# skit-ai/N-Best-ASR-Transformer

Measured on AMD Instinct MI355X. Metric: utterances/sec fine-tune (bert-base, seq128, n_best=5), higher is better.
Workload: dtype bf16

## Files before the change

include/nbest_hip.h:

```cpp
#ifndef NBEST_HIP_H
#define NBEST_HIP_H

#include <stddef.h>
#include <stdint.h>

#ifdef __cplusplus
extern "C" {
#endif

#define NBEST_ABI_VERSION 1

enum { NBEST_OK = 0, NBEST_ERR_ARG = -1, NBEST_ERR_SHAPE = -2, NBEST_ERR_DTYPE = -3, NBEST_ERR_ALIGN = -4,
       NBEST_ERR_LAUNCH = -5, NBEST_ERR_WORKSPACE = -6 };
enum { NBEST_F32 = 0, NBEST_BF16 = 1 };

typedef void* nbest_stream_t;

int nbest_version(void);
int nbest_last_error(char* buf, size_t n);

int nbest_embed_ln_fwd(const int64_t* ids, const int64_t* seg, const int64_t* pos, const void* word,
                       const void* type, const void* ptab, const float* gamma, const float* beta, void* out,
                       float* stats, int64_t M, int H, float eps, int dtype, float drop_p, uint64_t seed,
                       uint32_t drop_stream, nbest_stream_t stream);
int nbest_embed_ln_bwd(const int64_t* ids, const int64_t* seg, const int64_t* pos, const int32_t* perm, const void* word,
                       const void* type, const void* ptab, const float* gamma, const float* stats,
                       const void* dout, float* dword, float* dtype_tab, float* dptab, float* dgamma,
                       float* dbeta, int B, int S, int H, int n_types, int dtype, int64_t word_pad_id,
                       int64_t pos_pad_id, int accumulate, int tables_accumulate, float drop_p, uint64_t seed,
                       uint32_t drop_stream, void* ws, size_t ws_bytes, nbest_stream_t stream);
size_t nbest_embed_bwd_ws_bytes(int64_t M, int64_t H);
int nbest_embed_ln_fwd_interp(const int64_t* ids, const int64_t* base_ids, const float* alpha, const int64_t* seg, const int64_t* pos,
                              const void* word, const void* type, const void* ptab, const float* gamma, const float* beta, void* out,
                              float* stats, int B, int S, int H, float eps, int dtype, float drop_p, uint64_t seed, uint32_t drop_stream,
                              nbest_stream_t stream);
int nbest_embed_attrib(const int64_t* ids, const int64_t* base_ids, const float* alpha, const int64_t* seg, const int64_t* pos,
                       const void* word, const void* type, const void* ptab, const float* gamma, const void* dhidden, float* attr,
                       int pairs, int m, int S, int H, float eps, int dtype, nbest_stream_t stream);

int nbest_rows_gather(const float* table, const int64_t* rows, int64_t n_rows, int64_t cap, int64_t* ids_out, float* vals_out, int H,
                      nbest_stream_t stream);
int nbest_rows_zero(float* table, const int64_t* ids, int64_t n, int H, nbest_stream_t stream);
int nbest_rows_add(float* table, const int64_t* ids, const float* vals, int64_t n, int H, nbest_stream_t stream);

enum {
  NBEST_EPI_NONE = 0,
  NBEST_EPI_BIAS = 1,
  NBEST_EPI_BIAS_GELU = 2,
  NBEST_EPI_BIAS_DROP_RES = 3,
  NBEST_EPI_DGELU = 4,
  NBEST_EPI_RES = 5,
  NBEST_EPI_F32_SPLITK = 6
};
typedef struct nbest_gemm_args {
  const void* A;
  const void* B;
  void* C;
  const float* bias;
  const void* R;
  void* U;
  void* ws;
  size_t ws_bytes;
  int64_t M, N, K;
  int64_t lda, ldb, ldc, ldr, ldu;
  int32_t trans_a, trans_b;
  int32_t epilogue;
  int32_t dtype;
  int32_t accumulate;
  float drop_p;
  uint32_t drop_stream;
  uint64_t seed;
  float* colsum_out;
  int32_t colsum_accumulate;
  int32_t flags;
  const void* B_packed;
  int32_t b_pack_bn;
  int32_t pad_;
} nbest_gemm_args;
#define NBEST_GEMM_DEFER_REDUCE 1
size_t nbest_gemm_ws_bytes(const nbest_gemm_args* a);
int nbest_gemm(const nbest_gemm_args* a, nbest_stream_t stream);

size_t nbest_wgrad_pair_ws_bytes(const nbest_gemm_args* a, const nbest_gemm_args* b);
int nbest_wgrad_pair(const nbest_gemm_args* a, const nbest_gemm_args* b, nbest_stream_t stream);
int nbest_wgrad_group(const nbest_gemm_args* problems, int n, nbest_stream_t stream);

typedef struct nbest_gemm_fp8_args {
  const void* A;
  const void* B;
  void* C;
  const float* bias;
  const void* R;
  void* U;
  void* C8;
  int64_t M, N, K;
  int64_t lda, ldb, ldc, ldr, ldu, ldc8;
  int32_t epilogue;
  float out_scale;
  float drop_p;
  uint32_t drop_stream;
  uint64_t seed;
  const float* out_scale_dev;
  const uint32_t* a_amax;
  const uint32_t* c8_amax_prev;
  uint32_t* c8_amax_new;
  float* colsum_out;
  int32_t colsum_accumulate;
  int32_t pad;
  void* ws;
  size_t ws_bytes;
  const void* B_packed;
  int32_t b_pack_bn;
  int32_t pad3;
} nbest_gemm_fp8_args;
size_t nbest_gemm_fp8_ws_bytes(const nbest_gemm_fp8_args* a);
int nbest_gemm_fp8(const nbest_gemm_fp8_args* a, nbest_stream_t stream);
size_t nbest_wgrad_fp8_ws_bytes(int64_t M, int64_t N, int64_t K);
int nbest_wgrad_fp8(const void* dY8, const void* X8, float* dW, int64_t M, int64_t N, int64_t K, int64_t lda, int64_t ldb,
                    int64_t ldc, const uint32_t* a_amax, const uint32_t* x_amax, int accumulate, void* ws, size_t ws_bytes,
                    nbest_stream_t stream);
size_t nbest_wgrad_fp8_pair_ws_bytes(int64_t Ma, int64_t Mb, int64_t N, int64_t K);
int nbest_wgrad_fp8_pair(const void* dY8a, const void* X8a, float* dWa, int64_t Ma, int64_t lda_a, int64_t ldb_a, int64_t ldc_a,
                         const uint32_t* amax_a, const uint32_t* xamax_a, const void* dY8b, const void* X8b, float* dWb, int64_t Mb,
                         int64_t lda_b, int64_t ldb_b, int64_t ldc_b, const uint32_t* amax_b, const uint32_t* xamax_b, int64_t N, int64_t K,
                         int accumulate, void* ws, size_t ws_bytes, nbest_stream_t stream);
int nbest_cast_bf16_to_fp8(const void* src, void* dst, int64_t n, nbest_stream_t stream);

int nbest_attention_fwd(const void* qkv, const uint8_t* key_mask, void* ctx, float* lse, int B, int S,
                        int heads, int d, int dtype, float drop_p, uint64_t seed, uint32_t drop_stream,
                        nbest_stream_t stream);
int nbest_attention_cls_fwd(const void* q, int64_t ldq, const void* kv, int64_t ldkv, const uint8_t* key_mask, void* ctx,
                            int64_t ldctx, int B, int S, int heads, int d, int dtype, nbest_stream_t stream);
int nbest_attention_probs(const void* qkv, const uint8_t* key_mask, const float* lse, float* probs, int B, int S, int heads, int d,
                          int dtype, nbest_stream_t stream);
int nbest_attention_cls_probs(const void* q, int64_t ldq, const void* kv, int64_t ldkv, const uint8_t* key_mask, float* probs,
                              int64_t ldp, int B, int S, int heads, int d, int dtype, nbest_stream_t stream);
size_t nbest_attention_bwd_ws_bytes(int B, int S, int heads);
int nbest_attention_bwd(const void* qkv, const uint8_t* key_mask, const void* ctx, const void* dctx,
                        const float* lse, void* dqkv, float* dbias, int accumulate, void* ws, size_t ws_bytes,
                        int B, int S, int heads, int d, int dtype, float drop_p, uint64_t seed,
                        uint32_t drop_stream, nbest_stream_t stream);

size_t nbest_attention_keep_bytes(int B, int S, int heads);
int nbest_attention_fwd_keep(const void* qkv, const uint8_t* key_mask, void* ctx, float* lse, int B, int S,
                             int heads, int d, int dtype, float drop_p, uint64_t seed, uint32_t drop_stream,
                             void* keep, nbest_stream_t stream);
int nbest_attention_bwd_keep(const void* qkv, const uint8_t* key_mask, const void* ctx, const void* dctx,
                             const float* lse, void* dqkv, float* dbias, int accumulate, void* ws, size_t ws_bytes,
                             int B, int S, int heads, int d, int dtype, float drop_p, uint64_t seed,
                             uint32_t drop_stream, const void* keep, nbest_stream_t stream);

int nbest_layernorm_fwd(const void* x, const float* gamma, const float* beta, void* y, float* stats,
                        int64_t M, int H, float eps, int dtype, nbest_stream_t stream);
int nbest_layernorm_bwd(const void* dy, const void* x, const float* stats, const float* gamma, void* dx,
                        void* dx_drop, float* dgamma, float* dbeta, float* dbias, int64_t M, int H, int dtype,
                        int accumulate, float drop_p, uint64_t seed, uint32_t drop_stream, void* ws,
                        size_t ws_bytes, nbest_stream_t stream);
size_t nbest_rowred_ws_bytes(int64_t M, int64_t N);
int nbest_colsum(const void* X, float* out, int64_t M, int64_t N, int64_t ld, int dtype, int accumulate,
                 void* ws, size_t ws_bytes, nbest_stream_t stream);

typedef struct nbest_label_space {
  int32_t n_top, n_bottom, n_rows;
  const int32_t* bottom_off;
  const int32_t* bottom_ids;
  const int32_t* head_row;
} nbest_label_space;
size_t nbest_heads_ws_bytes(int B, int R, int H);
int nbest_stc_heads(const void* hidden, int64_t cls_stride, const float* Wh, const float* bh,
                    const nbest_label_space* ls, const float* labels, float* top, float* bott, float* final_scores,
                    float* loss_parts, float* dcls, float* dWh, float* dbh, int B, int H, int dtype,
                    int need_grad, int accumulate, float drop_p, uint64_t seed, uint32_t drop_stream, void* ws,
                    size_t ws_bytes, nbest_stream_t stream);
int nbest_stc_heads_vjp(const float* Wh, const nbest_label_space* ls, const float* top, const float* bott, const float* dtop,
                        const float* dbott, const float* dfin, float* dcls, float* dWh, float* dbh, int B, int H, int accumulate,
                        float drop_p, uint64_t seed, uint32_t drop_stream, void* ws, size_t ws_bytes, nbest_stream_t stream);

int nbest_cls_mse(const void* hidden_a, int64_t stride_a, const void* hidden_t, int64_t stride_t, float* loss,
                  float* da, float* dt, int B, int H, int dtype, float grad_scale, nbest_stream_t stream);

int nbest_cls_grad_scatter(const float* dcls, void* dhidden, int B, int S, int H, int dtype,
                           nbest_stream_t stream);

int nbest_stc_decode(const float* top, const float* bott, const nbest_label_space* ls,
                     const uint8_t* none_flag, int32_t* pred, int B, nbest_stream_t stream);
int nbest_stream_stamp(int32_t* flag, int32_t value, nbest_stream_t stream);

typedef struct nbest_tensor_desc {
  int64_t offset;
  int64_t numel;
  float lr;
  float wd;
  int32_t active;
  int32_t block_start;
} nbest_tensor_desc;
int nbest_bertadam_chunk(void);
int nbest_bertadam_step(float* p, float* g, float* m, float* v, void* p_lowp, const nbest_tensor_desc* descs,
                        int n_tensors, int n_blocks, float lr_mult, float b1, float b2, float eps,
                        float max_grad_norm, void* ws, size_t ws_bytes, nbest_stream_t stream);
int nbest_bertadam_norms(const float* g, const nbest_tensor_desc* descs, int n_tensors, int n_blocks, int blk_lo, int blk_hi,
                         float* partial, nbest_stream_t stream);
int nbest_bertadam_update(float* p, const float* g, float* m, float* v, void* p_lowp, const nbest_tensor_desc* descs,
                          int n_tensors, int n_blocks, int blk_lo, int blk_hi, const float* partial, float* coef,
                          float lr_mult, float b1, float b2, float eps, float max_grad_norm, nbest_stream_t stream);
enum { NBEST_ADAM_L2 = 0, NBEST_ADAMW = 1 };
int nbest_adam_clip_coef(const float* partial, int n_partial, float max_grad_norm, float* clip, nbest_stream_t stream);
int nbest_adam_update(int mode, float* p, const float* g, float* m, float* v, void* p_lowp, const nbest_tensor_desc* descs,
                      int n_tensors, int n_blocks, int blk_lo, int blk_hi, const float* clip, float lr_mult, float bc1,
                      float bc2_sqrt, double b1, double b2, float eps, nbest_stream_t stream);
int nbest_adam_step(int mode, float* p, float* g, float* m, float* v, void* p_lowp, const nbest_tensor_desc* descs,
                    int n_tensors, int n_blocks, float lr_mult, float bc1, float bc2_sqrt, double b1, double b2, float eps,
                    float max_grad_norm, void* ws, size_t ws_bytes, nbest_stream_t stream);
typedef struct nbest_matrix_desc {
  int64_t offset;
  int32_t rows, cols;
  int32_t tile_start, pad;
} nbest_matrix_desc;
#define NBEST_AMAX_TENSOR_WORDS 1024
int nbest_fp8_amax_fold(void* slots, void* out, int32_t n_tensors, nbest_stream_t stream);
int nbest_quantize_weights_fp8(const float* master, void* w8, void* w8t, const nbest_matrix_desc* descs, int n_matrices,
                               int n_tiles, float* inv_scale, void* ws, size_t ws_bytes, nbest_stream_t stream);
int nbest_transpose_weights(const void* src, void* dst, const nbest_matrix_desc* descs, int n_matrices, int n_tiles,
                            nbest_stream_t stream);
int nbest_pack_bn(int64_t N);
int nbest_pack_bn_fp8(int64_t N, int64_t K);
int nbest_pack_weights_fp8(const void* src, void* dst, const nbest_matrix_desc* descs, int n_matrices, int n_stages, nbest_stream_t stream);
int nbest_pack_weights(const void* src, void* dst, const nbest_matrix_desc* descs, int n_matrices, int n_stages, nbest_stream_t stream);
int nbest_cast_f32_to_bf16(const float* src, void* dst, int64_t n, nbest_stream_t stream);

typedef struct nbest_layer_offsets {
  int64_t wqkv, bqkv, wo, bo, ln1_g, ln1_b, w1, b1, w2, b2, ln2_g, ln2_b;
} nbest_layer_offsets;
typedef struct nbest_encoder_desc {
  int32_t dtype, B, S, H, L, heads, F;
  int32_t vocab, max_pos, n_types;
  float ln_eps, hidden_drop, attn_drop;
  int64_t word_pad_id, pos_pad_id;
  int64_t off_word, off_pos, off_type, off_emb_ln_g, off_emb_ln_b;
  const nbest_layer_offsets* layers_host;
  uint64_t seed;
  uint32_t drop_stream_base;
  int32_t wgrad_events_n;
  void** wgrad_events;
  const void* w8;
  const float* w8_inv_scale;
  const void* w8t;
  const uint32_t* gamax_prev;
  uint32_t* gamax_new;
  int32_t fp8_bwd;
  int32_t pad2;
  const void* wpk;
  const void* wpkt;
  const void* w8p;
  const void* w8tp;
  const int32_t* word_perm;
  const uint32_t* aamax_prev;
  uint32_t* aamax_new;
  int32_t fp8_act;
  int32_t pad4;
  int32_t first_trainable;
  int32_t no_input_grad;
  const uint8_t* wgrad_skip_host;
  const int64_t* base_ids;
  const float* alpha;
  int32_t no_param_grad;
  int32_t wgrad_group;
} nbest_encoder_desc;
enum { NBEST_WGRAD_GROUP_PLAN = 0, NBEST_WGRAD_GROUP_NEVER = 1, NBEST_WGRAD_GROUP_ALWAYS = 2 };
size_t nbest_encoder_act_bytes(const nbest_encoder_desc* d);
int nbest_encoder_act_view(const nbest_encoder_desc* d, void* act, int layer, void** qkv, float** lse);
size_t nbest_encoder_ws_bytes(const nbest_encoder_desc* d);
int nbest_encoder_wgrad_launches_per_layer(const nbest_encoder_desc* d);
int nbest_encoder_forward(const nbest_encoder_desc* d, const void* wts, const float* prm, const int64_t* ids,
                          const int64_t* seg, const int64_t* pos, const uint8_t* key_mask, void* act,
                          size_t act_bytes, void* ws, size_t ws_bytes, void** hidden_out, nbest_stream_t stream);
int nbest_encoder_backward(const nbest_encoder_desc* d, const void* wts, const void* wts_t, const float* prm, float* grad,
                           const int64_t* ids, const int64_t* seg, const int64_t* pos, const uint8_t* key_mask,
                           void* act, size_t act_bytes, void* dhidden, void* ws, size_t ws_bytes, int accumulate,
                           int layer_begin, int layer_end, int with_embeddings, nbest_stream_t stream);

size_t nbest_encoder_infer_ws_bytes(const nbest_encoder_desc* d);
int nbest_encoder_infer(const nbest_encoder_desc* d, const void* wts, const float* prm, const int64_t* ids, const int64_t* seg,
                        const int64_t* pos, const uint8_t* key_mask, void* ws, size_t ws_bytes, void* cls_out, nbest_stream_t stream);
int nbest_encoder_infer_attn(const nbest_encoder_desc* d, const void* wts, const float* prm, const int64_t* ids, const int64_t* seg,
                             const int64_t* pos, const uint8_t* key_mask, void* ws, size_t ws_bytes, void* cls_out, float* cls_attn,
                             nbest_stream_t stream);

#ifdef __cplusplus
}
#endif
#endif
```

n-best-asr-transformer_amd/arena.py:

```python
import ctypes as C

import torch

from . import hipabi as hb
from .synth import encoder_param_shapes, head_param_shapes

ALIGN = 64

NO_DECAY = ("bias", "LayerNorm.bias", "LayerNorm.weight")


class Slot:
    __slots__ = ("name", "shape", "offset", "numel")

    def __init__(self, name, shape, offset):
        self.name, self.shape, self.offset = name, tuple(shape), offset
        n = 1
        for s in shape:
            n *= s
        self.numel = n


class ParamArena:
    def __init__(self, cfg, labels, device, compute_dtype=torch.bfloat16):
        self.cfg, self.labels, self.device, self.compute_dtype = cfg, labels, torch.device(device), compute_dtype
        self.slots, self.by_name = [], {}
        off = 0

        def add(name, shape, align=True):
            nonlocal off
            if align:
                off = (off + ALIGN - 1) // ALIGN * ALIGN
            s = Slot(name, shape, off)
            self.slots.append(s)
            self.by_name[name] = s
            off += s.numel
            return s

        enc = dict(encoder_param_shapes(cfg))
        pre = "bert_encoder."
        for n in ("embeddings.word_embeddings.weight", "embeddings.position_embeddings.weight",
                  "embeddings.token_type_embeddings.weight", "embeddings.LayerNorm.weight", "embeddings.LayerNorm.bias"):
            add(pre + n, enc[n])
        self.layer_offsets = (hb.LayerOffsets * cfg.num_hidden_layers)()
        self.layer_range = []
        for i in range(cfg.num_hidden_layers):
            lp = "encoder.layer.%d." % i
            lo = None
            o = self.layer_offsets[i]
            for j, nm in enumerate(("query", "key", "value")):
                s = add(pre + lp + "attention.self.%s.weight" % nm, enc[lp + "attention.self.%s.weight" % nm], align=(j == 0))
                if j == 0:
                    o.wqkv, lo = s.offset, s.offset
            for j, nm in enumerate(("query", "key", "value")):
                s = add(pre + lp + "attention.self.%s.bias" % nm, enc[lp + "attention.self.%s.bias" % nm], align=(j == 0))
                if j == 0:
                    o.bqkv = s.offset
            for field, nm in (("wo", "attention.output.dense.weight"), ("bo", "attention.output.dense.bias"),
                              ("ln1_g", "attention.output.LayerNorm.weight"), ("ln1_b", "attention.output.LayerNorm.bias"),
                              ("w1", "intermediate.dense.weight"), ("b1", "intermediate.dense.bias"),
                              ("w2", "output.dense.weight"), ("b2", "output.dense.bias"),
                              ("ln2_g", "output.LayerNorm.weight"), ("ln2_b", "output.LayerNorm.bias")):
                setattr(o, field, add(pre + lp + nm, enc[lp + nm]).offset)
            self.layer_range.append((lo, off))
        add(pre + "pooler.dense.weight", enc["pooler.dense.weight"])
        add(pre + "pooler.dense.bias", enc["pooler.dense.bias"])
        heads = head_param_shapes(labels, cfg.hidden_size)
        w_names = [n for n, _ in heads if n.endswith("weight")]
        b_names = [n for n, _ in heads if n.endswith("bias")]
        hs = dict(heads)
        for j, n in enumerate(w_names):
            s = add("clf." + n, hs[n], align=(j == 0))
            if j == 0:
                self.off_wh = s.offset
        for j, n in enumerate(b_names):
            s = add("clf." + n, hs[n], align=(j == 0))
            if j == 0:
                self.off_bh = s.offset
        self.total = (off + ALIGN - 1) // ALIGN * ALIGN
        self.heads_range = (self.off_wh, off)
        self.emb_range = (0, self.layer_range[0][0]) if self.layer_range else (0, self.by_name[pre + "pooler.dense.weight"].offset)

        f32 = dict(dtype=torch.float32, device=self.device)
        self.p = torch.zeros(self.total, **f32)
        self.g = torch.zeros(self.total, **f32)
        self.m = None
        self.v = None
        self.w16 = torch.zeros(self.total, dtype=torch.bfloat16, device=self.device) if compute_dtype == torch.bfloat16 else None
        self.w16t = None
        self.lazy_w16t = False
        self.w16t_stale = False
        self.w8 = self.w8t = self.w8_inv_scale = self._w8_ws = self.gamax = self.aamax = self.gamax_slots = self.aamax_slots = None
        self._tdescs = None
        self.wpk = self.wpkt = None
        self.w8p = self.w8tp = None
        self._pdescs = None
        if self.w16 is not None and self.device.type == "cuda":
            self.w16t = torch.zeros(self.total, dtype=torch.bfloat16, device=self.device)
            H, F = cfg.hidden_size, cfg.intermediate_size
            mats = []
            for o in self.layer_offsets:
                mats += [(o.wqkv, 3 * H, H), (o.wo, H, H), (o.w1, F, H), (o.w2, H, F)]
            arr = (hb.MatrixDesc * len(mats))()
            t = 0
            for i, (off, r, c) in enumerate(mats):
                arr[i].offset, arr[i].rows, arr[i].cols, arr[i].tile_start = off, r, c, t
                t += ((r + 63) // 64) * ((c + 63) // 64)
            self._tdescs = (torch.frombuffer(bytearray(bytes(arr)), dtype=torch.uint8).to(self.device), len(mats), t)
            self._pdescs = []
            for transposed in (False, True):
                sel = []
                for off, r, c in mats:
                    n, k = (c, r) if transposed else (r, c)
                    bn = hb.lib().nbest_pack_bn(n)
                    if not (bn > 0 and k % 32 == 0 and n % bn == 0):
                        sel = None
                        break
                    sel.append((off, n, k, bn))
                if sel is None:
                    self._pdescs = None
                    break
                parr = (hb.MatrixDesc * len(sel))()
                t = 0
                for i, (off, n, k, bn) in enumerate(sel):
                    parr[i].offset, parr[i].rows, parr[i].cols, parr[i].tile_start, parr[i].pad = off, n, k, t, bn
                    t += (n // bn) * (k // 32)
                self._pdescs.append((torch.frombuffer(bytearray(bytes(parr)), dtype=torch.uint8).to(self.device), len(sel), t))
            if self._pdescs is not None:
                self.wpk = torch.zeros(self.total, dtype=torch.bfloat16, device=self.device)
                self.wpkt = torch.zeros(self.total, dtype=torch.bfloat16, device=self.device)
        self._descs = None

    def view(self, buf, name):
        s = self.by_name[name]
        return buf[s.offset:s.offset + s.numel].view(s.shape)

    def heads_wb(self):
        R, H = self.labels.n_head_rows, self.cfg.hidden_size
        return self.p[self.off_wh:self.off_wh + R * H].view(R, H), self.p[self.off_bh:self.off_bh + R]

    def heads_grad_wb(self):
        R, H = self.labels.n_head_rows, self.cfg.hidden_size
        return self.g[self.off_wh:self.off_wh + R * H].view(R, H), self.g[self.off_bh:self.off_bh + R]

    @property
    def weights(self):
        return self.w16 if self.w16 is not None else self.p

    def refresh_compute_copy(self):
        if self.w16 is not None:
            hb.cast_bf16(self.p, self.w16)
        self.refresh_transposed()

    def refresh_transposed(self):
        if self.w16t is not None:
            if self.lazy_w16t:
                self.w16t_stale = True
            else:
                self.refresh_w16t()
        if self.w8 is not None:
            d, n, t = self._tdescs
            hb.check(hb.lib().nbest_quantize_weights_fp8(hb.ptr(self.p), hb.ptr(self.w8), hb.ptr(self.w8t), hb.ptr(d), n, t,
                                                         hb.ptr(self.w8_inv_scale), hb.ptr(self._w8_ws), self._w8_ws.numel(),
                                                         hb.stream_ptr()), "quantize_weights_fp8")
            if getattr(self, "w8p", None) is not None:
                for src, dst, (pd, pn, pt) in ((self.w8, self.w8p, self._p8descs[0]), (self.w8t, self.w8tp, self._p8descs[1])):
                    hb.check(hb.lib().nbest_pack_weights_fp8(hb.ptr(src), hb.ptr(dst), hb.ptr(pd), pn, pt, hb.stream_ptr()), "pack_weights_fp8")

    def refresh_w16t(self):
        d, n, t = self._tdescs
        hb.check(hb.lib().nbest_transpose_weights(hb.ptr(self.w16), hb.ptr(self.w16t), hb.ptr(d), n, t, hb.stream_ptr()),
                 "transpose_weights")
        self.w16t_stale = False
        if self.wpk is not None:
            for src, dst, (pd, pn, pt) in ((self.w16, self.wpk, self._pdescs[0]), (self.w16t, self.wpkt, self._pdescs[1])):
                hb.check(hb.lib().nbest_pack_weights(hb.ptr(src), hb.ptr(dst), hb.ptr(pd), pn, pt, hb.stream_ptr()), "pack_weights")

    def enable_fp8_forward(self):
        if self.w16t is None:
            raise RuntimeError("nbest_amd: the fp8 forward needs the bf16 path on a GPU")
        self.wpk = self.wpkt = None
        if self.w8 is None:
            n = self._tdescs[1]
            self.w8 = torch.zeros(self.total, dtype=torch.uint8, device=self.device)
            self.w8t = torch.zeros(self.total, dtype=torch.uint8, device=self.device)
            self.gamax = torch.zeros(n, dtype=torch.int32, device=self.device)
            self.gamax_slots = torch.zeros(n * hb.AMAX_TENSOR_WORDS, dtype=torch.int32, device=self.device)
            self.aamax = torch.zeros(n, dtype=torch.int32, device=self.device)
            self.aamax_slots = torch.zeros(n * hb.AMAX_TENSOR_WORDS, dtype=torch.int32, device=self.device)
            self.w8_inv_scale = torch.ones(n, dtype=torch.float32, device=self.device)
            self._w8_ws = torch.zeros(4 * n + 16, dtype=torch.uint8, device=self.device)
            H, F = self.cfg.hidden_size, self.cfg.intermediate_size
            mats = []
            for o in self.layer_offsets:
                mats += [(o.wqkv, 3 * H, H), (o.wo, H, H), (o.w1, F, H), (o.w2, H, F)]
            self._p8descs = []
            for transposed in (False, True):
                parr = (hb.MatrixDesc * len(mats))()
                t = 0
                for i, (off, r, c) in enumerate(mats):
                    nn, kk = (c, r) if transposed else (r, c)
                    bn = hb.lib().nbest_pack_bn_fp8(nn, kk)
                    if not (bn > 0 and kk % 64 == 0 and nn % bn == 0):
                        parr = None
                        break
                    parr[i].offset, parr[i].rows, parr[i].cols, parr[i].tile_start, parr[i].pad = off, nn, kk, t, bn
                    t += (nn // bn) * (kk // 64)
                if parr is None:
                    self._p8descs = None
                    break
                self._p8descs.append((torch.frombuffer(bytearray(bytes(parr)), dtype=torch.uint8).to(self.device), len(mats), t))
            self.w8p = self.w8tp = None
            if self._p8descs is not None:
                self.w8p = torch.zeros(self.total, dtype=torch.uint8, device=self.device)
                self.w8tp = torch.zeros(self.total, dtype=torch.uint8, device=self.device)
            self.refresh_transposed()

    def load_state(self, sd, strict=True):
        missing = []
        for s in self.slots:
            if s.name in sd:
                src = sd[s.name]
                src = torch.as_tensor(src)
                if tuple(src.shape) != s.shape:
                    raise RuntimeError("shape mismatch for %s: %s vs %s" % (s.name, tuple(src.shape), s.shape))
                self.view(self.p, s.name).copy_(src.to(torch.float32))
            else:
                missing.append(s.name)
        if strict and missing:
            raise RuntimeError("missing keys: %s" % missing[:5])
        self.refresh_compute_copy()
        return missing

    def block_table(self, select=None, active=None):
        chunk = hb.lib().nbest_bertadam_chunk()
        out = []
        for s in self.slots:
            if select is not None and not select(s.name):
                continue
            act = 0 if "pooler" in s.name else 1
            if active is not None:
                act = int(bool(active(s.name)))
            for c0 in range(0, s.numel, chunk):
                out.append((s.offset + c0, min(chunk, s.numel - c0), act))
        return out

    def fp32_read_slots(self, select=None):
        return [s for s in self.slots if (select is None or select(s.name)) and "pooler" not in s.name and
                (s.name.startswith("clf.") or s.name.endswith("bias") or "LayerNorm" in s.name)]

    def build_descs(self, lr, bert_lr, active=None, select=None, wd=None):
        chunk = hb.lib().nbest_bertadam_chunk()
        slots = [s for s in self.slots if select is None or select(s.name)]
        n = len(slots)
        arr = (hb.TensorDesc * max(n, 1))()
        blk = 0
        for i, s in enumerate(slots):
            d = arr[i]
            d.offset, d.numel = s.offset, s.numel
            d.lr = bert_lr if "bert_encoder" in s.name else lr
            d.wd = 0.0 if any(nd in s.name for nd in NO_DECAY) else 0.01
            if wd is not None:
                d.wd = wd
            d.active = 0 if "pooler" in s.name else 1
            if active is not None:
                d.active = int(bool(active(s.name)))
            d.block_start = blk
            blk += (s.numel + chunk - 1) // chunk
        raw = bytes(arr)
        dev = torch.frombuffer(bytearray(raw), dtype=torch.uint8).to(self.device)
        return dev, n, blk
```

n-best-asr-transformer_amd/csrc/common.h:

```cpp
#pragma once
#include <hip/hip_runtime.h>
#include <stdint.h>
#include <math.h>

#include "../../include/nbest_hip.h"
#include "internal.h"

typedef __bf16 bf16;
typedef __attribute__((ext_vector_type(2))) __bf16 bf16x2;
typedef __attribute__((ext_vector_type(4))) __bf16 bf16x4;
typedef __attribute__((ext_vector_type(8))) __bf16 bf16x8;
typedef __attribute__((ext_vector_type(2))) float f32x2;
typedef __attribute__((ext_vector_type(4))) float f32x4;
typedef __attribute__((ext_vector_type(16))) float f32x16;
typedef __attribute__((ext_vector_type(4))) int i32x4;
typedef __attribute__((ext_vector_type(2))) int i32x2;

#define LDS_PTR(p) ((void __attribute__((address_space(3)))*)(p))

#define NB_CHECK(cond, code, ...)            \
  do {                                       \
    if (!(cond)) {                           \
      nbest_set_error(__VA_ARGS__);          \
      return (code);                         \
    }                                        \
  } while (0)
#define NB_LAUNCH_CHECK()                                                       \
  do {                                                                          \
    hipError_t e__ = hipGetLastError();                                         \
    if (e__ != hipSuccess) {                                                    \
      nbest_set_error("%s:%d launch failed: %s", __FILE__, __LINE__,            \
                      hipGetErrorString(e__));                                  \
      return NBEST_ERR_LAUNCH;                                                  \
    }                                                                           \
  } while (0)

static inline int64_t round_up(int64_t x, int64_t m) { return (x + m - 1) / m * m; }

constexpr int kEpiBiasGeluNoU = 0x102;
static inline int nb_kernel_epilogue(int epi, const void* U) { return (epi == NBEST_EPI_BIAS_GELU && !U) ? kEpiBiasGeluNoU : epi; }

template <typename T> __device__ __forceinline__ float to_f(T v);
template <> __device__ __forceinline__ float to_f<float>(float v) { return v; }
template <> __device__ __forceinline__ float to_f<bf16>(bf16 v) { return (float)v; }
template <typename T> __device__ __forceinline__ T from_f(float v);
template <> __device__ __forceinline__ float from_f<float>(float v) { return v; }
template <> __device__ __forceinline__ bf16 from_f<bf16>(float v) { return (bf16)v; }

template <typename T> struct Vec4;
template <> struct Vec4<float> {
  typedef f32x4 raw_t;
  static __device__ __forceinline__ raw_t raw_load(const float* p) { return *(const f32x4*)p; }
  static __device__ __forceinline__ f32x4 cvt(raw_t v) { return v; }
  static __device__ __forceinline__ f32x4 load(const float* p) { return *(const f32x4*)p; }
  static __device__ __forceinline__ void store(float* p, f32x4 v) { *(f32x4*)p = v; }
};
template <> struct Vec4<bf16> {
  typedef bf16x4 raw_t;
  static __device__ __forceinline__ raw_t raw_load(const bf16* p) { return *(const bf16x4*)p; }
  static __device__ __forceinline__ f32x4 cvt(raw_t v) { return f32x4{(float)v[0], (float)v[1], (float)v[2], (float)v[3]}; }
  static __device__ __forceinline__ f32x4 load(const bf16* p) {
    bf16x4 v = *(const bf16x4*)p;
    return f32x4{(float)v[0], (float)v[1], (float)v[2], (float)v[3]};
  }
  static __device__ __forceinline__ void store(bf16* p, f32x4 v) {
    bf16x4 o;
    o[0] = (bf16)v[0]; o[1] = (bf16)v[1]; o[2] = (bf16)v[2]; o[3] = (bf16)v[3];
    *(bf16x4*)p = o;
  }
};
template <typename T> struct Vec8;
template <> struct Vec8<float> {
  static __device__ __forceinline__ void load(const float* p, float* o) {
    f32x4 a = *(const f32x4*)p, b = *(const f32x4*)(p + 4);
    o[0] = a[0]; o[1] = a[1]; o[2] = a[2]; o[3] = a[3]; o[4] = b[0]; o[5] = b[1]; o[6] = b[2]; o[7] = b[3];
  }
  static __device__ __forceinline__ void store(float* p, const float* v) {
    *(f32x4*)p = f32x4{v[0], v[1], v[2], v[3]};
    *(f32x4*)(p + 4) = f32x4{v[4], v[5], v[6], v[7]};
  }
};
template <> struct Vec8<bf16> {
  static __device__ __forceinline__ void load(const bf16* p, float* o) {
    bf16x8 v = *(const bf16x8*)p;
#pragma unroll
    for (int i = 0; i < 8; ++i) o[i] = (float)v[i];
  }
  static __device__ __forceinline__ void store(bf16* p, const float* v) {
    bf16x8 o;
#pragma unroll
    for (int i = 0; i < 8; ++i) o[i] = (bf16)v[i];
    *(bf16x8*)p = o;
  }
};

__device__ __forceinline__ void nb_tile_coords(int t, int tiles_m, int gn, int& tm, int& tn) {
  const int per_group = tiles_m * gn;
  const int g = t / per_group, r = t - g * per_group;
  tm = r / gn;
  tn = g * gn + (r - tm * gn);
}
__device__ __forceinline__ int xcd_remap(int bid, int nwg) {
  const int q = nwg >> 3, r = nwg & 7, xcd = bid & 7, idx = bid >> 3;
  return (xcd < r ? xcd * (q + 1) : r * (q + 1) + (xcd - r) * q) + idx;
}
inline int nb_group_cols(int64_t tiles_n, int64_t slice_bytes_per_tile, int64_t limit_kb) {
  int best = 1;
  for (int d = 1; d <= tiles_n; ++d)
    if (tiles_n % d == 0 && d * slice_bytes_per_tile <= limit_kb * 1024) best = d;
  return best;
}

template <typename V> __device__ __forceinline__ void st_stream(V* p, V v, bool nt) {
  static_assert(sizeof(V) == 8 || sizeof(V) == 16, "st_stream: 8- or 16-byte vectors");
  (void)nt;
  __builtin_nontemporal_store(v, p);
}
__device__ __forceinline__ void st_stream_bf16x8(bf16* p, const float* v, bool nt) {
  bf16x8 o;
#pragma unroll
  for (int i = 0; i < 8; ++i) o[i] = (bf16)v[i];
  st_stream((bf16x8*)p, o, nt);
}
typedef unsigned int u32x4 __attribute__((ext_vector_type(4)));
typedef unsigned int u32x2 __attribute__((ext_vector_type(2)));
typedef unsigned int u32x3 __attribute__((ext_vector_type(3)));
__device__ __forceinline__ void nb_bstore_bf16x8(__amdgpu_buffer_rsrc_t rs, uint32_t byte_off, const float* v) {
  bf16x8 o;
#pragma unroll
  for (int i = 0; i < 8; ++i) o[i] = (bf16)v[i];
  __builtin_amdgcn_raw_buffer_store_b128(__builtin_bit_cast(u32x4, o), rs, byte_off, 0, 2 );
}
__device__ __forceinline__ void nb_bstore8(__amdgpu_buffer_rsrc_t rs, uint32_t byte_off, uint32_t lo, uint32_t hi) {
  __builtin_amdgcn_raw_buffer_store_b64(u32x2{lo, hi}, rs, byte_off, 0, 2 );
}

template <typename T>
__device__ __forceinline__ void transpose_tile64(const T* __restrict__ s, T* __restrict__ o, int rows, int cols, int r0, int c0,
                                                 T* tile) {
  constexpr int EPV = 16 / (int)sizeof(T);
  constexpr int PITCH = 64 + EPV;
  constexpr int CPR = 64 / EPV;
  typedef __attribute__((ext_vector_type(EPV))) T vec_t;
#pragma unroll
  for (int it = 0; it < (64 * CPR) / 256; ++it) {
    const int idx = it * 256 + threadIdx.x, r = idx / CPR, ch = idx % CPR;
    const vec_t v = *(const vec_t*)(s + (int64_t)(r0 + r) * cols + c0 + ch * EPV);
#pragma unroll
    for (int e = 0; e < EPV; ++e) tile[(ch * EPV + e) * PITCH + r] = v[e];
  }
  __syncthreads();
#pragma unroll
  for (int it = 0; it < (64 * CPR) / 256; ++it) {
    const int idx = it * 256 + threadIdx.x, c = idx / CPR, ch = idx % CPR;
    *(vec_t*)(o + (int64_t)(c0 + c) * rows + r0 + ch * EPV) = *(const vec_t*)(tile + c * PITCH + ch * EPV);
  }
}

__device__ __forceinline__ float wave_sum(float v) {
#pragma unroll
  for (int o = 32; o > 0; o >>= 1) v += __shfl_xor(v, o, 64);
  return v;
}
template <int CTRL> __device__ __forceinline__ float dpp_add(float v) {
  return v + __builtin_bit_cast(float, __builtin_amdgcn_update_dpp(0, __builtin_bit_cast(int, v), CTRL, 0xF, 0xF, true));
}
__device__ __forceinline__ void wave_sum2(float& a, float& b) {
  a = dpp_add<0xB1>(a); b = dpp_add<0xB1>(b);
  a = dpp_add<0x4E>(a); b = dpp_add<0x4E>(b);
  a = dpp_add<0x141>(a); b = dpp_add<0x141>(b);
  a = dpp_add<0x140>(a); b = dpp_add<0x140>(b);
  a += __shfl_xor(a, 16, 64); b += __shfl_xor(b, 16, 64);
  a += __shfl_xor(a, 32, 64); b += __shfl_xor(b, 32, 64);
}
__device__ __forceinline__ float wave_sum_dpp(float a) {
  a = dpp_add<0xB1>(a); a = dpp_add<0x4E>(a); a = dpp_add<0x141>(a); a = dpp_add<0x140>(a);
  a += __shfl_xor(a, 16, 64);
  a += __shfl_xor(a, 32, 64);
  return a;
}
__device__ __forceinline__ float wave_max(float v) {
#pragma unroll
  for (int o = 32; o > 0; o >>= 1) v = fmaxf(v, __shfl_xor(v, o, 64));
  return v;
}
__device__ __forceinline__ float block_sum(float v, float* smem) {
  v = wave_sum(v);
  const int w = threadIdx.x >> 6, nw = blockDim.x >> 6;
  __syncthreads();
  if ((threadIdx.x & 63) == 0) smem[w] = v;
  __syncthreads();
  float r = 0.f;
  for (int i = 0; i < nw; ++i) r += smem[i];
  return r;
}

__device__ __forceinline__ float gelu_f(float u) { return 0.5f * u * (1.0f + erff(u * 0.70710678118654752440f)); }
__device__ __forceinline__ float dgelu_f(float u) {
  const float cdf = 0.5f * (1.0f + erff(u * 0.70710678118654752440f));
  const float pdf = 0.39894228040143267794f * expf(-0.5f * u * u);
  return cdf + u * pdf;
}

__device__ __forceinline__ void gelu_parts_fast(float u, float& cdf, float& e) {
  const float z = fabsf(u) * 0.70710678118654752440f;
  const float t = __builtin_amdgcn_rcpf(fmaf(0.3275911f, z, 1.0f));
  float poly = fmaf(t, 1.061405429f, -1.453152027f);
  poly = fmaf(poly, t, 1.421413741f);
  poly = fmaf(poly, t, -0.284496736f);
  poly = fmaf(poly, t, 0.254829592f);
  e = __expf(-z * z);
  const float erf_abs = fmaf(-poly * t, e, 1.0f);
  cdf = fmaf(0.5f, copysignf(erf_abs, u), 0.5f);
}
__device__ __forceinline__ void gelu_pair_fast(f32x2 u, f32x2& h, f32x2& g) {
  const f32x2 au = {fabsf(u[0]), fabsf(u[1])};
  const f32x2 d = au * 0.23164190f + 1.0f;
  const f32x2 t = {__builtin_amdgcn_rcpf(d[0]), __builtin_amdgcn_rcpf(d[1])};
  f32x2 poly = t * (-0.5f * 1.061405429f) + (0.5f * 1.453152027f);
  poly = poly * t + (-0.5f * 1.421413741f);
  poly = poly * t + (0.5f * 0.284496736f);
  poly = poly * t + (-0.5f * 0.254829592f);
  const f32x2 x2 = (u * u) * (-0.5f * 1.4426950408889634f);
  const f32x2 e = {__builtin_amdgcn_exp2f(x2[0]), __builtin_amdgcn_exp2f(x2[1])};
  const f32x2 half_erf = (poly * t) * e + 0.5f;
  const f32x2 cdf = {0.5f + copysignf(half_erf[0], u[0]), 0.5f + copysignf(half_erf[1], u[1])};
  g = (u * 0.39894228040143267794f) * e + cdf;
  h = u * cdf;
}
__device__ __forceinline__ float gelu_fast(float u) {
  float cdf, e;
  gelu_parts_fast(u, cdf, e);
  return u * cdf;
}
__device__ __forceinline__ float dgelu_fast(float u) {
  float cdf, e;
  gelu_parts_fast(u, cdf, e);
  return fmaf(u * 0.39894228040143267794f, e, cdf);
}

__device__ __forceinline__ uint32_t gd_pack4(const float* g) {
  uint32_t w = 0;
#pragma unroll
  for (int e = 0; e < 4; ++e) w = __builtin_amdgcn_cvt_pk_u8_f32(fmaf(g[e], 200.f, 26.f), e, w);
  return w;
}
__device__ __forceinline__ void gd_unpack4(uint32_t w, float* g) {
#pragma unroll
  for (int e = 0; e < 4; ++e) g[e] = fmaf((float)((w >> (8 * e)) & 255u), 0.005f, -0.13f);
}

__device__ __forceinline__ uint32_t fp8_pack4(const float* v) {
  float c[4];
#pragma unroll
  for (int e = 0; e < 4; ++e) c[e] = __builtin_amdgcn_fmed3f(v[e], -448.f, 448.f);
  int w = 0;
  w = __builtin_amdgcn_cvt_pk_fp8_f32(c[0], c[1], w, false);
  w = __builtin_amdgcn_cvt_pk_fp8_f32(c[2], c[3], w, true);
  return (uint32_t)w;
}

struct Fp8Grad {
  uint8_t* out8;
  const uint32_t* amax_prev;
  uint32_t* amax_new;
};
__host__ __device__ __forceinline__ float fp8_pow2_scale(float amax, float target) {
  if (!(amax >= 7.8886e-31f) || !(amax <= 3.0e38f)) return 1.f;
  const float e = floorf(log2f(target / amax));
  return exp2f(e < -100.f ? -100.f : (e > 100.f ? 100.f : e));
}
__host__ __device__ __forceinline__ float fp8_scale_of(float amax) { return fp8_pow2_scale(amax, 224.f); }
__host__ __device__ __forceinline__ float fp8_gscale_of(float amax) { return fp8_pow2_scale(amax, 56.f); }
__device__ __forceinline__ float fp8_grad_scale(const uint32_t* amax_prev) { return amax_prev ? fp8_gscale_of(__uint_as_float(*amax_prev)) : 1.f; }
__host__ __device__ __forceinline__ float fp8_ascale_of(float amax) { return fp8_pow2_scale(amax, 224.f); }
__device__ __forceinline__ float fp8_act_scale(const uint32_t* amax_prev) { return amax_prev ? fp8_ascale_of(__uint_as_float(*amax_prev)) : 1.f; }
constexpr int kAmaxSlots = 16, kAmaxSlotStride = NBEST_AMAX_TENSOR_WORDS / 16;
__device__ __forceinline__ void amax_update(uint32_t* p, float v) {
  p += ((blockIdx.x + 5 * blockIdx.y + 3 * blockIdx.z) & (kAmaxSlots - 1)) * kAmaxSlotStride;
  const uint32_t b = __float_as_uint(v);
  if (b > __hip_atomic_load(p, __ATOMIC_RELAXED, __HIP_MEMORY_SCOPE_AGENT)) atomicMax(p, b);
}

__device__ __forceinline__ uint32_t nb_hash32(uint32_t x) {
  x ^= x >> 16; x *= 0x7feb352dU; x ^= x >> 15; x *= 0x846ca68bU; x ^= x >> 16;
  return x;
}
struct DropCfg {
  uint32_t thr16;
  float scale;
  uint32_t key;
};
__host__ __device__ __forceinline__ uint32_t nb_mix_key(uint64_t seed, uint32_t stream) {
  uint64_t z = seed + 0x9E3779B97F4A7C15ULL * (uint64_t)(stream + 1);
  z = (z ^ (z >> 30)) * 0xBF58476D1CE4E5B9ULL;
  z = (z ^ (z >> 27)) * 0x94D049BB133111EBULL;
  return (uint32_t)(z ^ (z >> 31));
}
__device__ __forceinline__ bool nb_keep(const DropCfg& d, uint32_t idx) {
  const uint32_t h = nb_hash32((idx >> 1) * 0x9E3779B9U + d.key);
  const uint32_t u = (idx & 1) ? (h >> 16) : (h & 0xFFFFu);
  return u >= d.thr16;
}
__device__ __forceinline__ uint32_t nb_keep2(const DropCfg& d, uint32_t idx) {
  const uint32_t h = nb_hash32((idx >> 1) * 0x9E3779B9U + d.key);
  return ((h & 0xFFFFu) >= d.thr16 ? 1u : 0u) | ((h >> 16) >= d.thr16 ? 2u : 0u);
}
__device__ __forceinline__ uint32_t nb_keep4(const DropCfg& d, uint32_t idx) {
  const uint32_t h0 = nb_hash32((idx >> 1) * 0x9E3779B9U + d.key);
  const uint32_t h1 = nb_hash32(((idx >> 1) + 1) * 0x9E3779B9U + d.key);
  return ((h0 & 0xFFFFu) >= d.thr16 ? 1u : 0u) | ((h0 >> 16) >= d.thr16 ? 2u : 0u) |
         ((h1 & 0xFFFFu) >= d.thr16 ? 4u : 0u) | ((h1 >> 16) >= d.thr16 ? 8u : 0u);
}
static inline DropCfg make_drop(float p, uint64_t seed, uint32_t stream) {
  DropCfg d;
  uint32_t thr = (p <= 0.f) ? 0u : (uint32_t)lrintf(p * 65536.0f);
  if (thr > 65535u) thr = 65535u;
  d.thr16 = thr;
  d.scale = 65536.0f / (float)(65536u - thr);
  d.key = nb_mix_key(seed, stream);
  return d;
}
```

n-best-asr-transformer_amd/csrc/gemm_bf16_v2.hip:

```cpp
#include "common.h"
#include <type_traits>

namespace {

constexpr int BK = 32;

struct GemmP2 {
  const bf16* A; const bf16* B; void* C; const float* bias; const bf16* R; bf16* U; float* slab; float* colpart;
  int64_t M, N, K, lda, ldb, ldc, ldr, ldu;
  int64_t k_per_split;
  int tiles_m, tiles_n, splits, accumulate;
  uint32_t a_bytes, b_bytes;
  uint32_t c_bytes, r_bytes, u_bytes;
  DropCfg drop;
  int stream_out;
  int gn;
  const bf16* A2; const bf16* B2;
  int64_t lda2, ldb2, m_split;
  uint32_t a2_bytes, b2_bytes;
  const bf16* Bp;
  uint32_t bp_bytes;
  int bp_bn;
};

// ... 785 lines not shown
  }
}

template <int BM, int BN, int WM, int WN, int STAGES, bool TA, bool TB, int EPI>
__global__ __launch_bounds__(WM * WN * 64, 2) void gemm2_kernel(GemmP2 p) {
  gemm2_body<BM, BN, WM, WN, STAGES, TA, TB, EPI>(p, xcd_remap(blockIdx.x, gridDim.x));
}

constexpr int kMaxGroup = 8;
struct WgradProb {
  const bf16* A; const bf16* B; float* C;
  int64_t lda, ldb, ldc;
  uint32_t a_bytes, b_bytes;
  int tiles_m, tiles_n, gn, tile_start;
};
struct WgradGroupP {
  WgradProb pr[kMaxGroup];
  int64_t K, k_pad;
  int n, accumulate;
};

template <int BM, int BN, int WM, int WN, int STAGES, bool TA, bool TB, int EPI>
__global__ __launch_bounds__(WM * WN * 64, 2) void gemm2_kernel_grouped(WgradGroupP g) {
  static_assert(BM == 256 && BN == 256 && TA && TB && EPI == NBEST_EPI_F32_SPLITK, "grouped launch: the 256 x 256 weight-gradient program only");
  const int id = xcd_remap(blockIdx.x, gridDim.x);
  WgradProb q = g.pr[0];
#pragma unroll
  for (int i = 1; i < kMaxGroup; ++i)
    if (i < g.n && id >= g.pr[i].tile_start) q = g.pr[i];
  GemmP2 p = {};
  p.A = q.A; p.B = q.B; p.C = q.C;
  p.M = (int64_t)q.tiles_m * 256; p.N = (int64_t)q.tiles_n * 256; p.K = g.K;
  p.lda = q.lda; p.ldb = q.ldb; p.ldc = q.ldc;
  p.k_per_split = g.k_pad;
  p.tiles_m = q.tiles_m; p.tiles_n = q.tiles_n; p.splits = 1; p.accumulate = g.accumulate;
  p.a_bytes = q.a_bytes; p.b_bytes = q.b_bytes;
  p.stream_out = 1;
  p.gn = q.gn;
  gemm2_body<BM, BN, WM, WN, STAGES, TA, TB, EPI>(p, id - q.tile_start);
}

__global__ __launch_bounds__(256) void pack_b_kernel(const bf16* __restrict__ src, bf16* __restrict__ dst,
                                                     const nbest_matrix_desc* __restrict__ descs, int n) {
  int lo = 0, hi = n - 1;
  while (lo < hi) {
    const int mid = (lo + hi + 1) >> 1;
    if (descs[mid].tile_start <= (int)blockIdx.x) lo = mid; else hi = mid - 1;
  }
  const nbest_matrix_desc d = descs[lo];
  const int bn = d.pad, pw = (bn == 256) ? 128 : 96;
  const int nk = d.cols / BK, t = blockIdx.x - d.tile_start, tile_n = t / nk, kt = t - tile_n * nk;
  const bf16* s = src + d.offset + ((int64_t)tile_n * bn) * d.cols + (int64_t)kt * BK;
  bf16* o = dst + d.offset + ((int64_t)tile_n * nk + kt) * bn * BK;
  for (int p = threadIdx.x; p < bn * 4; p += blockDim.x) {
    const int row = p >> 2, slot = p & 3;
    const int kc = slot ^ ((-(row >> 2)) & 3);
    const int x = row % pw;
    const int grow = row - x + (pw / 16) * (x & 15) + (x >> 4);
    *(i32x4*)(o + (int64_t)p * 8) = *(const i32x4*)(s + (int64_t)grow * d.cols + kc * 8);
  }
}

struct Plan {
  int bm, bn, splits;
  int64_t kps;
};

static Plan make_plan(const nbest_gemm_args* a) {
  Plan pl;
  pl.bn = 128;
  const int64_t t256 = ((a->M + 255) / 256) * (a->N / 128);
  pl.bm = (!a->trans_a && t256 >= 1024) ? 256 : 128;
  const bool ok256 = (a->N % 256 == 0) && (!a->trans_a || a->M % 256 == 0);
  if (!a->trans_a && !a->trans_b && a->N % 256 == 0 &&
      [&] {
        const int64_t t = ((a->M + 255) / 256) * (a->N / 256);
        return t >= 1024 || (t >= 256 && (double)t / (double)(((t + 255) / 256) * 256) >= 0.85);
      }()) {
    pl.bm = 256; pl.bn = 256;
  } else if (a->trans_a && a->trans_b && a->epilogue == NBEST_EPI_F32_SPLITK && ok256 && (a->M / 256) * (a->N / 256) >= 18) {
    pl.bm = 256; pl.bn = 256;
  }
  {
    const bool epi192 = a->epilogue == NBEST_EPI_NONE || a->epilogue == NBEST_EPI_BIAS || a->epilogue == NBEST_EPI_BIAS_DROP_RES ||
                        a->epilogue == NBEST_EPI_RES;
    if (!a->trans_a && !a->trans_b && a->N % 192 == 0 && epi192) {
      const int64_t rows = (a->M + 255) / 256, t192 = rows * (a->N / 192);
      auto eff = [](int64_t t) { return (double)t / (double)(((t + 255) / 256) * 256); };
      const double e256 = (a->N % 256 == 0) ? eff(rows * (a->N / 256)) : 0.0;
      if (t192 >= 256 && 0.85 * eff(t192) > e256) { pl.bm = 256; pl.bn = 192; }
    }
    if (pl.bm == 256 && pl.bn == 192 && a->N % 384 == 0 && a->K % BK == 0) { pl.bm = 128; pl.bn = 384; }
    if (pl.bm == 256 && pl.bn == 256 && !a->trans_a && !a->trans_b && epi192 && a->N % 512 == 0 && a->N <= 2048 && a->K % BK == 0) { pl.bm = 128; pl.bn = 512; }
  }
  const int64_t tiles = ((a->M + pl.bm - 1) / pl.bm) * (a->N / pl.bn);
  const int64_t slots = (pl.bn >= 192) ? 256 : 512;
  pl.splits = 1;
  pl.kps = round_up(a->K, 64);
  if (a->epilogue == NBEST_EPI_F32_SPLITK) nb_splitk_plan(tiles, a->K, slots, (4 * slots + 4) / 5, &pl.splits, &pl.kps);
  return pl;
}

template <int BM, int BN, int WM, int WN, int STAGES, bool TA, bool TB>
static int launch2(const GemmP2& p, int epi, int grid, hipStream_t st) {
  constexpr int NT = WM * WN * 64;
  constexpr int lds_bytes = STAGES * (BM + BN) * BK * 2 + (((BN * 4) % NT) ? (NT / 64) * 1024 : 0);
#define L(E)                                                                                                        \
  case E:                                                                                                           \
    (void)hipFuncSetAttribute((const void*)gemm2_kernel<BM, BN, WM, WN, STAGES, TA, TB, E>, hipFuncAttributeMaxDynamicSharedMemorySize, lds_bytes); \
    gemm2_kernel<BM, BN, WM, WN, STAGES, TA, TB, E><<<grid, NT, lds_bytes, st>>>(p);                                 \
    break;
  if constexpr (BN / WN == 64) {
    if (epi == NBEST_EPI_F32_SPLITK) {
      switch (epi) { L(NBEST_EPI_F32_SPLITK) }
      NB_LAUNCH_CHECK();
      return NBEST_OK;
    }
  }
  if constexpr (BN / WN == 96) {
    switch (epi) {
      L(NBEST_EPI_NONE) L(NBEST_EPI_BIAS) L(NBEST_EPI_BIAS_DROP_RES) L(NBEST_EPI_RES)
      default:
        nbest_set_error("gemm: epilogue %d is not built for 192-column tiles", epi);
        return NBEST_ERR_ARG;
    }
  } else {
    switch (epi) {
      L(NBEST_EPI_NONE) L(NBEST_EPI_BIAS) L(NBEST_EPI_BIAS_GELU) L(NBEST_EPI_BIAS_DROP_RES) L(NBEST_EPI_DGELU)
      L(NBEST_EPI_RES) L(kEpiBiasGeluNoU)
      default:
        nbest_set_error("gemm: bad epilogue %d", epi);
        return NBEST_ERR_ARG;
    }
  }
#undef L
  NB_LAUNCH_CHECK();
  return NBEST_OK;
}

}

bool nbest_gemm_bf16_v2_wins(const nbest_gemm_args* a) {
  if (a->colsum_out && a->epilogue != NBEST_EPI_DGELU && a->epilogue != NBEST_EPI_F32_SPLITK && !a->trans_a && !a->trans_b) return false;
  const Plan pl = make_plan(a);
  return pl.bm == 256 || (pl.bm == 128 && pl.bn >= 384);
}

size_t nbest_gemm_bf16_v2_ws_bytes(const nbest_gemm_args* a) {
  if (a->epilogue != NBEST_EPI_F32_SPLITK) {
    if (!a->colsum_out) return 0;
    const Plan pl0 = make_plan(a);
    return (size_t)((a->M + pl0.bm - 1) / pl0.bm) * 4 * a->N * sizeof(float);
  }
  const Plan pl = make_plan(a);
  return pl.splits > 1 ? (size_t)pl.splits * a->M * a->N * sizeof(float) : 0;
}

static int gemm_v2_impl(const nbest_gemm_args* a, const nbest_gemm_args* b2, int64_t m_split, hipStream_t st) {
  NB_CHECK(a->N % 64 == 0, NBEST_ERR_SHAPE, "gemm(bf16): N=%lld must be a multiple of 64", (long long)a->N);
  NB_CHECK(a->trans_a || a->K % BK == 0, NBEST_ERR_SHAPE, "gemm(bf16): K=%lld must be a multiple of %d", (long long)a->K, BK);
  const Plan pl = make_plan(a);
  GemmP2 p;
  p.A = (const bf16*)a->A; p.B = (const bf16*)a->B; p.C = a->C; p.bias = a->bias; p.R = (const bf16*)a->R; p.U = (bf16*)a->U;
  p.M = a->M; p.N = a->N; p.K = a->K; p.lda = a->lda; p.ldb = a->ldb; p.ldc = a->ldc; p.ldr = a->ldr; p.ldu = a->ldu;
  p.tiles_m = (int)((a->M + pl.bm - 1) / pl.bm);
  p.tiles_n = (int)(a->N / pl.bn);
  p.splits = pl.splits;
  p.k_per_split = pl.kps;
  p.accumulate = a->accumulate;
  p.slab = (float*)a->ws;
  p.colpart = nullptr;
  p.A2 = p.B2 = nullptr; p.lda2 = p.ldb2 = p.m_split = 0; p.a2_bytes = p.b2_bytes = 0;
  p.Bp = nullptr; p.bp_bytes = 0; p.bp_bn = 0;
  if (a->B_packed && ((a->b_pack_bn == pl.bn && pl.bm == 256 && (pl.bn == 256 || pl.bn == 192)) || (pl.bm == 128 && pl.bn == 384 && a->b_pack_bn == 192) || (pl.bm == 128 && pl.bn == 512 && a->b_pack_bn == 256)) &&
      !a->trans_a && !a->trans_b &&
      a->epilogue != NBEST_EPI_F32_SPLITK && a->K % BK == 0 && a->N * a->K * 2 < ((int64_t)1 << 32) && ((uintptr_t)a->B_packed & 15) == 0) {
    p.Bp = (const bf16*)a->B_packed;
    p.bp_bytes = (uint32_t)(a->N * a->K * 2);
    p.bp_bn = a->b_pack_bn;
  }
  if (a->colsum_out && a->epilogue != NBEST_EPI_F32_SPLITK) {
    NB_CHECK(a->epilogue == NBEST_EPI_DGELU || a->trans_a || a->trans_b, NBEST_ERR_ARG,
             "gemm(bf16, generation 2): column sums are fused into the x GELU' epilogue only (nbest_gemm routes the others to generation 1)");
    NB_CHECK(a->ws && a->ws_bytes >= nbest_gemm_bf16_v2_ws_bytes(a), NBEST_ERR_WORKSPACE, "gemm: column-sum workspace too small");
    p.colpart = (float*)a->ws;
  }
  const int64_t a_rows = a->trans_a ? a->K : a->M, a_cols = a->trans_a ? (b2 ? m_split : a->M) : a->K;
  const int64_t b_rows = a->trans_b ? a->K : a->N, b_cols = a->trans_b ? a->N : a->K;
  const int64_t ab = ((a_rows - 1) * a->lda + a_cols) * 2, bb = ((b_rows - 1) * a->ldb + b_cols) * 2;
  p.a_bytes = (uint32_t)ab; p.b_bytes = (uint32_t)bb;
  if (b2) {
    const int64_t ab2 = ((a->K - 1) * b2->lda + b2->M) * 2, bb2 = ((a->K - 1) * b2->ldb + a->N) * 2;
    p.A2 = (const bf16*)b2->A; p.B2 = (const bf16*)b2->B; p.lda2 = b2->lda; p.ldb2 = b2->ldb; p.m_split = m_split;
    p.a2_bytes = (uint32_t)ab2; p.b2_bytes = (uint32_t)bb2;
    NB_CHECK(pl.bm == 256 && pl.bn == 256 && pl.splits > 1 && m_split % 256 == 0, NBEST_ERR_SHAPE, "wgrad pair: not a 256 x 256 split-K plan");
  }
  p.c_bytes = p.r_bytes = p.u_bytes = 0;
  if (a->epilogue != NBEST_EPI_F32_SPLITK) {
    const int64_t mpad = a->M + 256;
    NB_CHECK(mpad * a->ldc * 2 < ((int64_t)1 << 32) && mpad * a->ldr * 2 < ((int64_t)1 << 32) && mpad * a->ldu < ((int64_t)1 << 32),
             NBEST_ERR_SHAPE, "gemm(bf16): output / residual larger than 4 GiB");
    p.c_bytes = (uint32_t)(a->M * a->ldc * 2);
    p.r_bytes = a->R ? (uint32_t)(a->M * a->ldr * 2) : 0;
    p.u_bytes = a->U ? (uint32_t)(a->M * a->ldu) : 0;
  }
  p.drop = make_drop(a->drop_p, a->seed, a->drop_stream);
  p.stream_out = 1;
  p.gn = (!a->trans_a && !a->trans_b) ? nb_group_cols(a->N / pl.bn, (int64_t)pl.bn * a->K * 2, 2400) : (int)(a->N / pl.bn);
  if (pl.bm == 128 && pl.bn >= 384 && (a->N / pl.bn) % 2 == 0) p.gn = 2;
  const int epi = a->epilogue;
  if (epi == NBEST_EPI_F32_SPLITK && p.splits > 1)
    NB_CHECK(a->ws && a->ws_bytes >= (size_t)p.splits * a->M * a->N * sizeof(float), NBEST_ERR_WORKSPACE,
             "gemm: split-K workspace too small (%zu < %zu)", a->ws_bytes, (size_t)p.splits * a->M * a->N * sizeof(float));
  const int grid = p.tiles_m * p.tiles_n * p.splits;
  const int kepi = nb_kernel_epilogue(epi, a->U);
  int rc, wave_rows = 2;
  NB_CHECK(a->N % pl.bn == 0, NBEST_ERR_SHAPE, "gemm(bf16): N=%lld is not a multiple of the %d-column tile", (long long)a->N, pl.bn);
  if (pl.bm == 128 && pl.bn == 512) {
    rc = launch2<128, 512, 2, 4, 4, false, false>(p, kepi, grid, st);
  } else if (pl.bm == 128 && pl.bn == 384) {
    if (a->K >= 2048) rc = launch2<128, 384, 2, 4, 5, false, false>(p, kepi, grid, st);
    else rc = launch2<128, 384, 2, 4, 4, false, false>(p, kepi, grid, st);
  } else if (pl.bm == 256 && pl.bn == 192) {
    if (a->K >= 2048) rc = launch2<256, 192, 4, 2, 5, false, false>(p, kepi, grid, st);
    else rc = launch2<256, 192, 4, 2, 4, false, false>(p, kepi, grid, st);
    wave_rows = 4;
  } else if (pl.bm == 256 && pl.bn == 256) {
    if (!a->trans_a && !a->trans_b && epi != NBEST_EPI_F32_SPLITK) {
      if (a->K >= 2048) rc = launch2<256, 256, 4, 2, 5, false, false>(p, kepi, grid, st);
      else rc = launch2<256, 256, 4, 2, 4, false, false>(p, kepi, grid, st);
      wave_rows = 4;
    }
    else if (!a->trans_a && !a->trans_b) rc = launch2<256, 256, 2, 4, 4, false, false>(p, kepi, grid, st);
    else if (!a->trans_a && a->trans_b) rc = launch2<256, 256, 2, 4, 4, false, true>(p, kepi, grid, st);
    else rc = launch2<256, 256, 2, 4, 4, true, true>(p, kepi, grid, st);
  } else if (pl.bm == 256) {
    if (!a->trans_b && epi != NBEST_EPI_F32_SPLITK) { rc = launch2<256, 128, 4, 1, 3, false, false>(p, kepi, grid, st); wave_rows = 4; }
    else if (!a->trans_b) rc = launch2<256, 128, 2, 2, 3, false, false>(p, kepi, grid, st);
    else rc = launch2<256, 128, 2, 2, 3, false, true>(p, kepi, grid, st);
  } else {
    nbest_set_error("gemm(bf16, generation 2): no kernel for the %d x %d plan", pl.bm, pl.bn);
    return NBEST_ERR_SHAPE;
  }
  if (rc) return rc;
  if (p.colpart) return nbest_internal_partial_rows_sum(p.colpart, p.tiles_m * wave_rows, (int)a->N, a->colsum_out, a->colsum_accumulate, st);
  if (epi == NBEST_EPI_F32_SPLITK && p.splits > 1 && !(a->flags & NBEST_GEMM_DEFER_REDUCE))
    return nbest_internal_splitk_reduce(p.slab, (float*)a->C, a->M, a->N, a->ldc, p.splits, a->accumulate, b2 ? (float*)b2->C : nullptr,
                                        b2 ? m_split : a->M, b2 ? b2->ldc : 0, st);
  return NBEST_OK;
}

int nbest_gemm_bf16_v2(const nbest_gemm_args* a, hipStream_t st) { return gemm_v2_impl(a, nullptr, 0, st); }

static bool pair_virtual(const nbest_gemm_args* a, const nbest_gemm_args* b, nbest_gemm_args* v) {
  if (a->dtype != NBEST_BF16 || b->dtype != NBEST_BF16 || !a->trans_a || !a->trans_b || !b->trans_a || !b->trans_b) return false;
  if (a->epilogue != NBEST_EPI_F32_SPLITK || b->epilogue != NBEST_EPI_F32_SPLITK) return false;
  if (a->N != b->N || a->K != b->K || a->accumulate != b->accumulate || a->M % 256 || b->M % 256 || a->N % 256) return false;
  if ((a->flags | b->flags) & NBEST_GEMM_DEFER_REDUCE) return false;
  *v = *a;
  v->M = a->M + b->M;
  const Plan pl = make_plan(v);
  return pl.bm == 256 && pl.bn == 256 && pl.splits > 1;
}
size_t nbest_wgrad_pair_bf16_ws_bytes(const nbest_gemm_args* a, const nbest_gemm_args* b) {
  nbest_gemm_args v;
  if (!pair_virtual(a, b, &v)) return 0;
  return nbest_gemm_bf16_v2_ws_bytes(&v);
}
int nbest_wgrad_pair_bf16(const nbest_gemm_args* a, const nbest_gemm_args* b, hipStream_t st) {
  nbest_gemm_args v;
  NB_CHECK(pair_virtual(a, b, &v), NBEST_ERR_SHAPE, "wgrad pair: the two problems do not share one 256 x 256 split-K launch");
  return gemm_v2_impl(&v, b, a->M, st);
}

int nbest_wgrad_group_bf16(const nbest_gemm_args* pr, int n, hipStream_t st) {
  NB_CHECK(n >= 1 && n <= kMaxGroup, NBEST_ERR_ARG, "wgrad_group: %d problems (1 .. %d)", n, kMaxGroup);
  WgradGroupP g = {};
  g.n = n; g.K = pr[0].K; g.k_pad = round_up(pr[0].K, 64); g.accumulate = pr[0].accumulate;
  int tiles = 0;
  for (int i = 0; i < n; ++i) {
    const nbest_gemm_args* a = pr + i;
    NB_CHECK(a->dtype == NBEST_BF16 && a->trans_a && a->trans_b && a->epilogue == NBEST_EPI_F32_SPLITK, NBEST_ERR_ARG,
             "wgrad_group: problem %d is not a bf16 weight gradient (trans_a = trans_b = 1, NBEST_EPI_F32_SPLITK)", i);
    NB_CHECK(a->M % 256 == 0 && a->N % 256 == 0, NBEST_ERR_SHAPE, "wgrad_group: problem %d: %lld x %lld is not a multiple of the 256 x 256 tile", i,
             (long long)a->M, (long long)a->N);
    NB_CHECK(a->K == g.K && a->accumulate == g.accumulate, NBEST_ERR_ARG, "wgrad_group: problem %d differs in K or accumulate", i);
    WgradProb& q = g.pr[i];
    q.A = (const bf16*)a->A; q.B = (const bf16*)a->B; q.C = (float*)a->C;
    q.lda = a->lda; q.ldb = a->ldb; q.ldc = a->ldc;
    q.a_bytes = (uint32_t)(((a->K - 1) * a->lda + a->M) * 2); q.b_bytes = (uint32_t)(((a->K - 1) * a->ldb + a->N) * 2);
    q.tiles_m = (int)(a->M / 256); q.tiles_n = (int)(a->N / 256);
    q.gn = (q.tiles_n > q.tiles_m && q.tiles_n % 3 == 0) ? 3 : q.tiles_n;
    q.tile_start = tiles;
    tiles += q.tiles_m * q.tiles_n;
  }
  constexpr int lds_bytes = 4 * (256 + 256) * BK * 2;
  const auto kernel = gemm2_kernel_grouped<256, 256, 2, 4, 4, true, true, NBEST_EPI_F32_SPLITK>;
  (void)hipFuncSetAttribute((const void*)kernel, hipFuncAttributeMaxDynamicSharedMemorySize, lds_bytes);
  kernel<<<tiles, 512, lds_bytes, st>>>(g);
  NB_LAUNCH_CHECK();
  return NBEST_OK;
}

int nbest_pack_bn_internal(int64_t N) {
  if (N % 256 == 0 && N >= 1024) return 256;
  if (N % 192 == 0) return 192;
  return 0;
}

int nbest_pack_weights_bf16(const void* src, void* dst, const nbest_matrix_desc* descs, int n_matrices, int n_stages, hipStream_t st) {
  pack_b_kernel<<<n_stages, 256, 0, st>>>((const bf16*)src, (bf16*)dst, descs, n_matrices);
  NB_LAUNCH_CHECK();
  return NBEST_OK;
}
```

n-best-asr-transformer_amd/csrc/optim.hip:

```cpp
#include "common.h"

namespace {

constexpr int kChunk = 16384;

__device__ __forceinline__ int find_tensor(const nbest_tensor_desc* __restrict__ d, int n, int blk) {
  int lo = 0, hi = n - 1;
  while (lo < hi) {
    const int mid = (lo + hi + 1) >> 1;
    if (d[mid].block_start <= blk) lo = mid; else hi = mid - 1;
  }
  return lo;
}

__global__ __launch_bounds__(256) void sumsq_kernel(const float* __restrict__ g, const nbest_tensor_desc* __restrict__ descs,
                                                    int n_tensors, float* __restrict__ partial, int blk_off) {
  __shared__ float sm[16];
  const int blk = blockIdx.x + blk_off;
  const int t = find_tensor(descs, n_tensors, blk);
  const nbest_tensor_desc d = descs[t];
  float s = 0.f;
  if (d.active) {
    const int64_t c0 = (int64_t)(blk - d.block_start) * kChunk;
    const int64_t c1 = (c0 + kChunk < d.numel) ? c0 + kChunk : d.numel;
    const float* gp = g + d.offset;
    const bool vec = ((d.offset & 3) == 0);
    if (vec) {
      const int64_t v1 = c0 + ((c1 - c0) & ~(int64_t)3);
      for (int64_t i = c0 + 4 * threadIdx.x; i < v1; i += 1024) {
        f32x4 x = *(const f32x4*)(gp + i);
        s += (x[0] * x[0] + x[1] * x[1]) + (x[2] * x[2] + x[3] * x[3]);
      }
      for (int64_t i = v1 + threadIdx.x; i < c1; i += 256) s += gp[i] * gp[i];
    } else {
      for (int64_t i = c0 + threadIdx.x; i < c1; i += 256) s += gp[i] * gp[i];
    }
  }
  s = block_sum(s, sm);
  if (threadIdx.x == 0) partial[blk] = s;
}

__global__ __launch_bounds__(64) void clip_coef_kernel(const float* __restrict__ partial, const nbest_tensor_desc* __restrict__ descs,
                                                       int n_tensors, int n_blocks, float max_norm, float* __restrict__ coef) {
  const int t = blockIdx.x;
  const int b0 = descs[t].block_start;
  const int b1 = (t + 1 < n_tensors) ? descs[t + 1].block_start : n_blocks;
  float s = 0.f;
  for (int b = b0 + threadIdx.x; b < b1; b += 64) s += partial[b];
  s = wave_sum(s);
  if (threadIdx.x == 0) {
    float c = 1.f;
    if (max_norm > 0.f) c = fminf(max_norm / (sqrtf(s) + 1e-6f), 1.0f);
    coef[t] = c;
  }
}

__device__ __forceinline__ void adam1(float& p, float g, float& m, float& v, float coef, float b1, float b2, float eps,
                                      float lr, float wd) {
  g *= coef;
  m = m * b1 + (1.f - b1) * g;
  v = v * b2 + (1.f - b2) * g * g;
  float u = m / (sqrtf(v) + eps);
  if (wd > 0.f) u += wd * p;
  p -= lr * u;
}

__global__ __launch_bounds__(256) void bertadam_kernel(float* __restrict__ p, const float* __restrict__ g, float* __restrict__ m,
                                                       float* __restrict__ v, bf16* __restrict__ plow,
                                                       const nbest_tensor_desc* __restrict__ descs, int n_tensors,
                                                       const float* __restrict__ coef, float lr_mult, float b1, float b2, float eps,
                                                       int blk_off) {
  const int blk = blockIdx.x + blk_off;
  const int t = find_tensor(descs, n_tensors, blk);
  const nbest_tensor_desc d = descs[t];
  if (!d.active) return;
  const float cf = coef[t];
  const float lr = d.lr * lr_mult;
  const int64_t c0 = (int64_t)(blk - d.block_start) * kChunk;
  const int64_t c1 = (c0 + kChunk < d.numel) ? c0 + kChunk : d.numel;
  const int64_t base = d.offset;
  const bool vec = ((base & 3) == 0);
  int64_t v1 = c0;
  if (vec) {
    v1 = c0 + ((c1 - c0) & ~(int64_t)3);
    for (int64_t i = c0 + 4 * threadIdx.x; i < v1; i += 1024) {
      f32x4 pp = *(f32x4*)(p + base + i), gg = *(const f32x4*)(g + base + i);
      f32x4 mm = *(f32x4*)(m + base + i), vv = *(f32x4*)(v + base + i);
#pragma unroll
      for (int e = 0; e < 4; ++e) {
        float p1 = pp[e], m1 = mm[e], v1e = vv[e];
        adam1(p1, gg[e], m1, v1e, cf, b1, b2, eps, lr, d.wd);
        pp[e] = p1; mm[e] = m1; vv[e] = v1e;
      }
      *(f32x4*)(p + base + i) = pp;
      *(f32x4*)(m + base + i) = mm;
      *(f32x4*)(v + base + i) = vv;
      if (plow) Vec4<bf16>::store(plow + base + i, pp);
    }
  }
  for (int64_t i = v1 + threadIdx.x; i < c1; i += 256) {
    float pp = p[base + i], mm = m[base + i], vv = v[base + i];
    adam1(pp, g[base + i], mm, vv, cf, b1, b2, eps, lr, d.wd);
    p[base + i] = pp; m[base + i] = mm; v[base + i] = vv;
    if (plow) plow[base + i] = (bf16)pp;
  }
}

__global__ __launch_bounds__(256) void global_clip_kernel(const float* __restrict__ partial, int n, float max_norm,
                                                          float* __restrict__ out) {
  __shared__ double sm[256];
  double s = 0.0;
  for (int i = threadIdx.x; i < n; i += 256) s += (double)partial[i];
  sm[threadIdx.x] = s;
  __syncthreads();
#pragma unroll
  for (int w = 128; w > 0; w >>= 1) {
    if ((int)threadIdx.x < w) sm[threadIdx.x] += sm[threadIdx.x + w];
    __syncthreads();
  }
  if (threadIdx.x == 0) {
    const float total = (float)sqrt(sm[0]);
    float c = 1.f;
    if (max_norm > 0.f) c = fminf(max_norm / (total + 1e-6f), 1.0f);
    out[0] = c;
    out[1] = total;
  }
}

template <int MODE>
__device__ __forceinline__ void adam_mode1(float& p, float g, float& m, float& v, float c, float b1, float b2, float ob1, float ob2,
                                           float eps, float lr, float wd, float bc2s) {
  g *= c;
  if (MODE == NBEST_ADAM_L2) {
    if (wd != 0.f) g += wd * p;
    m += ob1 * (g - m);
    v = v * b2 + ob2 * g * g;
    p += -lr * (m / (sqrtf(v) / bc2s + eps));
  } else {
    m = m * b1 + ob1 * g;
    v = v * b2 + ob2 * g * g;
    p += -lr * (m / (sqrtf(v) + eps));
    if (wd > 0.f) p += (-lr * wd) * p;
  }
}

template <int MODE>
__global__ __launch_bounds__(256) void adam_kernel(float* __restrict__ p, const float* __restrict__ g, float* __restrict__ m,
                                                   float* __restrict__ v, bf16* __restrict__ plow,
                                                   const nbest_tensor_desc* __restrict__ descs, int n_tensors,
                                                   const float* __restrict__ clip, float lr_mult, float bc1, float bc2s, float b1,
                                                   float b2, float ob1, float ob2, float eps, int blk_off) {
  const int blk = blockIdx.x + blk_off;
  const int t = find_tensor(descs, n_tensors, blk);
  const nbest_tensor_desc d = descs[t];
  if (!d.active) return;
  const float cf = clip[0];
  const float lr = d.lr * lr_mult / bc1;
  const int64_t c0 = (int64_t)(blk - d.block_start) * kChunk;
  const int64_t c1 = (c0 + kChunk < d.numel) ? c0 + kChunk : d.numel;
  const int64_t base = d.offset;
  const bool vec = ((base & 3) == 0);
  int64_t v1 = c0;
  if (vec) {
    v1 = c0 + ((c1 - c0) & ~(int64_t)3);
    for (int64_t i = c0 + 4 * threadIdx.x; i < v1; i += 1024) {
      f32x4 pp = *(f32x4*)(p + base + i), gg = *(const f32x4*)(g + base + i);
      f32x4 mm = *(f32x4*)(m + base + i), vv = *(f32x4*)(v + base + i);
#pragma unroll
      for (int e = 0; e < 4; ++e) {
        float p1 = pp[e], m1 = mm[e], v1e = vv[e];
        adam_mode1<MODE>(p1, gg[e], m1, v1e, cf, b1, b2, ob1, ob2, eps, lr, d.wd, bc2s);
        pp[e] = p1; mm[e] = m1; vv[e] = v1e;
      }
      *(f32x4*)(p + base + i) = pp;
      *(f32x4*)(m + base + i) = mm;
      *(f32x4*)(v + base + i) = vv;
      if (plow) Vec4<bf16>::store(plow + base + i, pp);
    }
  }
  for (int64_t i = v1 + threadIdx.x; i < c1; i += 256) {
    float pp = p[base + i], mm = m[base + i], vv = v[base + i];
    adam_mode1<MODE>(pp, g[base + i], mm, vv, cf, b1, b2, ob1, ob2, eps, lr, d.wd, bc2s);
    p[base + i] = pp; m[base + i] = mm; v[base + i] = vv;
    if (plow) plow[base + i] = (bf16)pp;
  }
}

__global__ __launch_bounds__(256) void transpose_multi_kernel(const bf16* __restrict__ src, bf16* __restrict__ dst,
                                                              const nbest_matrix_desc* __restrict__ descs, int n) {
  __shared__ __attribute__((aligned(16))) bf16 tile[64][72];
  int lo = 0, hi = n - 1;
  while (lo < hi) {
    const int mid = (lo + hi + 1) >> 1;
    if (descs[mid].tile_start <= (int)blockIdx.x) lo = mid; else hi = mid - 1;
  }
  const nbest_matrix_desc d = descs[lo];
  const int t = blockIdx.x - d.tile_start, tc = (d.cols + 63) / 64;
  const int r0 = (t / tc) * 64, c0 = (t % tc) * 64;
  const int tx = threadIdx.x & 63, ty = threadIdx.x >> 6;
  const bf16* s = src + d.offset;
  bf16* o = dst + d.offset;
  if (r0 + 64 <= d.rows && c0 + 64 <= d.cols && ((d.rows | d.cols | d.offset) & 7) == 0) {
    transpose_tile64<bf16>(s, o, d.rows, d.cols, r0, c0, &tile[0][0]);
    return;
  }
#pragma unroll
  for (int i = 0; i < 16; ++i) {
    const int r = r0 + ty + 4 * i, c = c0 + tx;
    tile[ty + 4 * i][tx] = (r < d.rows && c < d.cols) ? s[(int64_t)r * d.cols + c] : (bf16)0.f;
  }
  __syncthreads();
#pragma unroll
  for (int i = 0; i < 16; ++i) {
    const int c = c0 + ty + 4 * i, r = r0 + tx;
    if (c < d.cols && r < d.rows) o[(int64_t)c * d.rows + r] = tile[tx][ty + 4 * i];
  }
}

}

extern "C" int nbest_transpose_weights(const void* src, void* dst, const nbest_matrix_desc* descs, int n_matrices, int n_tiles,
                                       nbest_stream_t stream) {
  NB_CHECK(src && dst && descs && n_matrices > 0 && n_tiles > 0, NBEST_ERR_ARG, "transpose_weights: bad arguments");
  transpose_multi_kernel<<<n_tiles, 256, 0, (hipStream_t)stream>>>((const bf16*)src, (bf16*)dst, descs, n_matrices);
  NB_LAUNCH_CHECK();
  return NBEST_OK;
}

extern "C" int nbest_bertadam_chunk(void) { return kChunk; }

extern "C" int nbest_bertadam_norms(const float* g, const nbest_tensor_desc* descs, int n_tensors, int n_blocks, int blk_lo, int blk_hi,
                                    float* partial, nbest_stream_t stream) {
  NB_CHECK(g && descs && partial && n_tensors > 0 && 0 <= blk_lo && blk_lo <= blk_hi && blk_hi <= n_blocks, NBEST_ERR_ARG,
           "bertadam_norms: bad arguments");
  if (blk_hi == blk_lo) return NBEST_OK;
  sumsq_kernel<<<blk_hi - blk_lo, 256, 0, (hipStream_t)stream>>>(g, descs, n_tensors, partial, blk_lo);
  NB_LAUNCH_CHECK();
  return NBEST_OK;
}

extern "C" int nbest_bertadam_update(float* p, const float* g, float* m, float* v, void* p_lowp, const nbest_tensor_desc* descs,
                                     int n_tensors, int n_blocks, int blk_lo, int blk_hi, const float* partial, float* coef,
                                     float lr_mult, float b1, float b2, float eps, float max_grad_norm, nbest_stream_t stream) {
  NB_CHECK(p && g && m && v && descs && partial && coef && n_tensors > 0 && 0 <= blk_lo && blk_lo <= blk_hi && blk_hi <= n_blocks,
           NBEST_ERR_ARG, "bertadam_update: bad arguments");
  hipStream_t st = (hipStream_t)stream;
  clip_coef_kernel<<<n_tensors, 64, 0, st>>>(partial, descs, n_tensors, n_blocks, max_grad_norm, coef);
  NB_LAUNCH_CHECK();
  if (blk_hi == blk_lo) return NBEST_OK;
  bertadam_kernel<<<blk_hi - blk_lo, 256, 0, st>>>(p, g, m, v, (bf16*)p_lowp, descs, n_tensors, coef, lr_mult, b1, b2, eps, blk_lo);
  NB_LAUNCH_CHECK();
  return NBEST_OK;
}

extern "C" int nbest_bertadam_step(float* p, float* g, float* m, float* v, void* p_lowp, const nbest_tensor_desc* descs,
                                   int n_tensors, int n_blocks, float lr_mult, float b1, float b2, float eps, float max_grad_norm,
                                   void* ws, size_t ws_bytes, nbest_stream_t stream) {
  NB_CHECK(p && g && m && v && descs && ws && n_tensors > 0 && n_blocks > 0, NBEST_ERR_ARG, "bertadam: null pointer");
  NB_CHECK(ws_bytes >= ((size_t)n_blocks + n_tensors) * sizeof(float), NBEST_ERR_WORKSPACE, "bertadam: workspace too small");
  float* partial = (float*)ws;
  float* coef = partial + n_blocks;
  if (int rc = nbest_bertadam_norms(g, descs, n_tensors, n_blocks, 0, n_blocks, partial, stream)) return rc;
  return nbest_bertadam_update(p, g, m, v, p_lowp, descs, n_tensors, n_blocks, 0, n_blocks, partial, coef, lr_mult, b1, b2, eps,
                               max_grad_norm, stream);
}

extern "C" int nbest_adam_clip_coef(const float* partial, int n_partial, float max_grad_norm, float* clip, nbest_stream_t stream) {
  NB_CHECK(partial && clip && n_partial > 0, NBEST_ERR_ARG, "adam_clip_coef: bad arguments");
  global_clip_kernel<<<1, 256, 0, (hipStream_t)stream>>>(partial, n_partial, max_grad_norm, clip);
  NB_LAUNCH_CHECK();
  return NBEST_OK;
}

extern "C" int nbest_adam_update(int mode, float* p, const float* g, float* m, float* v, void* p_lowp, const nbest_tensor_desc* descs,
                                 int n_tensors, int n_blocks, int blk_lo, int blk_hi, const float* clip, float lr_mult, float bc1,
                                 float bc2_sqrt, double b1, double b2, float eps, nbest_stream_t stream) {
  NB_CHECK(p && g && m && v && descs && clip && n_tensors > 0 && 0 <= blk_lo && blk_lo <= blk_hi && blk_hi <= n_blocks &&
           (mode == NBEST_ADAM_L2 || mode == NBEST_ADAMW) && bc1 > 0.f && bc2_sqrt > 0.f, NBEST_ERR_ARG, "adam_update: bad arguments");
  if (blk_hi == blk_lo) return NBEST_OK;
  hipStream_t st = (hipStream_t)stream;
  const float fb1 = (float)b1, fb2 = (float)b2, ob1 = (float)(1.0 - b1), ob2 = (float)(1.0 - b2);
  if (mode == NBEST_ADAM_L2)
    adam_kernel<NBEST_ADAM_L2><<<blk_hi - blk_lo, 256, 0, st>>>(p, g, m, v, (bf16*)p_lowp, descs, n_tensors, clip, lr_mult, bc1,
                                                                bc2_sqrt, fb1, fb2, ob1, ob2, eps, blk_lo);
  else
    adam_kernel<NBEST_ADAMW><<<blk_hi - blk_lo, 256, 0, st>>>(p, g, m, v, (bf16*)p_lowp, descs, n_tensors, clip, lr_mult, bc1,
                                                              bc2_sqrt, fb1, fb2, ob1, ob2, eps, blk_lo);
  NB_LAUNCH_CHECK();
  return NBEST_OK;
}

extern "C" int nbest_adam_step(int mode, float* p, float* g, float* m, float* v, void* p_lowp, const nbest_tensor_desc* descs,
                               int n_tensors, int n_blocks, float lr_mult, float bc1, float bc2_sqrt, double b1, double b2, float eps,
                               float max_grad_norm, void* ws, size_t ws_bytes, nbest_stream_t stream) {
  NB_CHECK(p && g && m && v && descs && ws && n_tensors > 0 && n_blocks > 0, NBEST_ERR_ARG, "adam_step: null pointer");
  NB_CHECK(ws_bytes >= ((size_t)n_blocks + 2) * sizeof(float), NBEST_ERR_WORKSPACE, "adam_step: workspace too small");
  float* partial = (float*)ws;
  float* clip = partial + n_blocks;
  if (int rc = nbest_bertadam_norms(g, descs, n_tensors, n_blocks, 0, n_blocks, partial, stream)) return rc;
  if (int rc = nbest_adam_clip_coef(partial, n_blocks, max_grad_norm, clip, stream)) return rc;
  return nbest_adam_update(mode, p, g, m, v, p_lowp, descs, n_tensors, n_blocks, 0, n_blocks, clip, lr_mult, bc1, bc2_sqrt, b1, b2, eps,
                           stream);
}
```

n-best-asr-transformer_amd/hipabi.py:

```python
import ctypes as C
import os

import torch

_HERE = os.path.dirname(os.path.abspath(__file__))
LIB_PATH = os.environ.get("NBEST_LIB") or os.path.join(_HERE, "csrc", "libnbest_hip.so")

F32, BF16 = 0, 1
ADAM_L2, ADAMW = 0, 1
EPI_NONE, EPI_BIAS, EPI_BIAS_GELU, EPI_BIAS_DROP_RES, EPI_DGELU, EPI_RES, EPI_F32_SPLITK = range(7)

EXPORTS = [
    "nbest_version", "nbest_last_error", "nbest_embed_ln_fwd", "nbest_embed_ln_bwd", "nbest_embed_bwd_ws_bytes", "nbest_rows_gather", "nbest_rows_zero", "nbest_rows_add",
    "nbest_gemm_ws_bytes", "nbest_gemm", "nbest_wgrad_pair_ws_bytes", "nbest_wgrad_pair", "nbest_wgrad_group", "nbest_pack_bn", "nbest_pack_weights", "nbest_pack_bn_fp8", "nbest_pack_weights_fp8", "nbest_attention_fwd", "nbest_attention_bwd", "nbest_attention_bwd_ws_bytes", "nbest_attention_keep_bytes", "nbest_attention_fwd_keep", "nbest_attention_bwd_keep", "nbest_layernorm_fwd",
    "nbest_layernorm_bwd", "nbest_rowred_ws_bytes", "nbest_colsum", "nbest_heads_ws_bytes", "nbest_stc_heads",
    "nbest_stc_heads_vjp", "nbest_cls_mse", "nbest_cls_grad_scatter", "nbest_stc_decode", "nbest_stream_stamp", "nbest_fp8_amax_fold", "nbest_bertadam_chunk", "nbest_bertadam_step", "nbest_bertadam_norms", "nbest_bertadam_update",
    "nbest_adam_clip_coef", "nbest_adam_update", "nbest_adam_step",
    "nbest_cast_f32_to_bf16", "nbest_transpose_weights", "nbest_encoder_act_bytes", "nbest_encoder_ws_bytes", "nbest_encoder_wgrad_launches_per_layer", "nbest_encoder_forward",
    "nbest_encoder_backward", "nbest_gemm_fp8", "nbest_gemm_fp8_ws_bytes", "nbest_wgrad_fp8", "nbest_wgrad_fp8_ws_bytes", "nbest_wgrad_fp8_pair", "nbest_wgrad_fp8_pair_ws_bytes", "nbest_cast_bf16_to_fp8", "nbest_quantize_weights_fp8",
    "nbest_attention_cls_fwd", "nbest_encoder_infer_ws_bytes", "nbest_encoder_infer",
    "nbest_attention_probs", "nbest_attention_cls_probs", "nbest_encoder_act_view", "nbest_encoder_infer_attn",
    "nbest_embed_ln_fwd_interp", "nbest_embed_attrib",
]


class GemmArgs(C.Structure):
    _fields_ = [("A", C.c_void_p), ("B", C.c_void_p), ("C", C.c_void_p), ("bias", C.c_void_p), ("R", C.c_void_p),
                ("U", C.c_void_p), ("ws", C.c_void_p), ("ws_bytes", C.c_size_t),
                ("M", C.c_int64), ("N", C.c_int64), ("K", C.c_int64),
                ("lda", C.c_int64), ("ldb", C.c_int64), ("ldc", C.c_int64), ("ldr", C.c_int64), ("ldu", C.c_int64),
                ("trans_a", C.c_int32), ("trans_b", C.c_int32), ("epilogue", C.c_int32), ("dtype", C.c_int32),
                ("accumulate", C.c_int32), ("drop_p", C.c_float), ("drop_stream", C.c_uint32), ("seed", C.c_uint64),
                ("colsum_out", C.c_void_p), ("colsum_accumulate", C.c_int32), ("flags", C.c_int32),
                ("B_packed", C.c_void_p), ("b_pack_bn", C.c_int32), ("pad_", C.c_int32)]


class GemmFp8Args(C.Structure):
    _fields_ = [("A", C.c_void_p), ("B", C.c_void_p), ("C", C.c_void_p), ("bias", C.c_void_p), ("R", C.c_void_p), ("U", C.c_void_p),
                ("C8", C.c_void_p), ("M", C.c_int64), ("N", C.c_int64), ("K", C.c_int64),
                ("lda", C.c_int64), ("ldb", C.c_int64), ("ldc", C.c_int64), ("ldr", C.c_int64), ("ldu", C.c_int64), ("ldc8", C.c_int64),
                ("epilogue", C.c_int32), ("out_scale", C.c_float), ("drop_p", C.c_float), ("drop_stream", C.c_uint32), ("seed", C.c_uint64),
                ("out_scale_dev", C.c_void_p), ("a_amax", C.c_void_p), ("c8_amax_prev", C.c_void_p), ("c8_amax_new", C.c_void_p),
                ("colsum_out", C.c_void_p), ("colsum_accumulate", C.c_int32), ("pad", C.c_int32), ("ws", C.c_void_p), ("ws_bytes", C.c_size_t),
                ("B_packed", C.c_void_p), ("b_pack_bn", C.c_int32), ("pad3", C.c_int32)]


class LabelSpaceC(C.Structure):
    _fields_ = [("n_top", C.c_int32), ("n_bottom", C.c_int32), ("n_rows", C.c_int32),
                ("bottom_off", C.c_void_p), ("bottom_ids", C.c_void_p), ("head_row", C.c_void_p)]


class TensorDesc(C.Structure):
    _fields_ = [("offset", C.c_int64), ("numel", C.c_int64), ("lr", C.c_float), ("wd", C.c_float),
                ("active", C.c_int32), ("block_start", C.c_int32)]


class MatrixDesc(C.Structure):
    _fields_ = [("offset", C.c_int64), ("rows", C.c_int32), ("cols", C.c_int32), ("tile_start", C.c_int32), ("pad", C.c_int32)]


class LayerOffsets(C.Structure):
    _fields_ = [(n, C.c_int64) for n in ("wqkv", "bqkv", "wo", "bo", "ln1_g", "ln1_b", "w1", "b1", "w2", "b2", "ln2_g", "ln2_b")]


class EncoderDesc(C.Structure):
    _fields_ = [("dtype", C.c_int32), ("B", C.c_int32), ("S", C.c_int32), ("H", C.c_int32), ("L", C.c_int32),
                ("heads", C.c_int32), ("F", C.c_int32), ("vocab", C.c_int32), ("max_pos", C.c_int32), ("n_types", C.c_int32),
                ("ln_eps", C.c_float), ("hidden_drop", C.c_float), ("attn_drop", C.c_float),
                ("word_pad_id", C.c_int64), ("pos_pad_id", C.c_int64),
                ("off_word", C.c_int64), ("off_pos", C.c_int64), ("off_type", C.c_int64),
                ("off_emb_ln_g", C.c_int64), ("off_emb_ln_b", C.c_int64),
                ("layers_host", C.POINTER(LayerOffsets)), ("seed", C.c_uint64), ("drop_stream_base", C.c_uint32),
                ("wgrad_events_n", C.c_int32), ("wgrad_events", C.POINTER(C.c_void_p)),
                ("w8", C.c_void_p), ("w8_inv_scale", C.c_void_p), ("w8t", C.c_void_p), ("gamax_prev", C.c_void_p),
                ("gamax_new", C.c_void_p), ("fp8_bwd", C.c_int32), ("pad2", C.c_int32),
                ("wpk", C.c_void_p), ("wpkt", C.c_void_p), ("w8p", C.c_void_p), ("w8tp", C.c_void_p),
                ("word_perm", C.c_void_p), ("aamax_prev", C.c_void_p), ("aamax_new", C.c_void_p), ("fp8_act", C.c_int32), ("pad4", C.c_int32),
                ("first_trainable", C.c_int32), ("no_input_grad", C.c_int32), ("wgrad_skip_host", C.c_void_p),
                ("base_ids", C.c_void_p), ("alpha", C.c_void_p), ("no_param_grad", C.c_int32), ("pad5", C.c_int32)]
    wgrad_group = property(lambda self: self.pad5, lambda self, v: setattr(self, "pad5", int(v)))


_lib = None


def lib():
    global _lib
    if _lib is None:
        if not os.path.exists(LIB_PATH):
            raise RuntimeError("nbest_amd: %s is missing - build it with `make -C %s` (hipcc, gfx950). "
                               "There is no CPU fallback for the product path." % (LIB_PATH, os.path.dirname(LIB_PATH)))
        L = C.CDLL(LIB_PATH)
        for name in EXPORTS:
            if not hasattr(L, name):
                raise RuntimeError("nbest_amd: %s does not export %s" % (LIB_PATH, name))
        for name in ("nbest_embed_bwd_ws_bytes", "nbest_gemm_ws_bytes", "nbest_wgrad_pair_ws_bytes", "nbest_rowred_ws_bytes", "nbest_heads_ws_bytes",
                     "nbest_attention_bwd_ws_bytes", "nbest_attention_keep_bytes",
                     "nbest_encoder_act_bytes", "nbest_encoder_ws_bytes", "nbest_encoder_infer_ws_bytes"):
            getattr(L, name).restype = C.c_size_t
        L.nbest_embed_bwd_ws_bytes.argtypes = [C.c_int64, C.c_int64]
        L.nbest_rows_gather.argtypes = [C.c_void_p, C.c_void_p, C.c_int64, C.c_int64, C.c_void_p, C.c_void_p, C.c_int, C.c_void_p]
        L.nbest_rows_zero.argtypes = [C.c_void_p, C.c_void_p, C.c_int64, C.c_int, C.c_void_p]
        L.nbest_rows_add.argtypes = [C.c_void_p, C.c_void_p, C.c_void_p, C.c_int64, C.c_int, C.c_void_p]
        L.nbest_rowred_ws_bytes.argtypes = [C.c_int64, C.c_int64]
        L.nbest_heads_ws_bytes.argtypes = [C.c_int, C.c_int, C.c_int]
        L.nbest_gemm_ws_bytes.argtypes = [C.POINTER(GemmArgs)]
        L.nbest_gemm.argtypes = [C.POINTER(GemmArgs), C.c_void_p]
        L.nbest_wgrad_pair_ws_bytes.argtypes = [C.POINTER(GemmArgs), C.POINTER(GemmArgs)]
        L.nbest_wgrad_pair.argtypes = [C.POINTER(GemmArgs), C.POINTER(GemmArgs), C.c_void_p]
        L.nbest_wgrad_group.argtypes = [C.POINTER(GemmArgs), C.c_int32, C.c_void_p]
        L.nbest_encoder_act_bytes.argtypes = [C.POINTER(EncoderDesc)]
        L.nbest_encoder_ws_bytes.argtypes = [C.POINTER(EncoderDesc)]
        L.nbest_encoder_wgrad_launches_per_layer.argtypes = [C.POINTER(EncoderDesc)]
        vp, i64, i32, f32, u64, u32, sz = C.c_void_p, C.c_int64, C.c_int, C.c_float, C.c_uint64, C.c_uint32, C.c_size_t
        L.nbest_embed_ln_fwd.argtypes = [vp] * 10 + [i64, i32, f32, i32, f32, u64, u32, vp]
        L.nbest_embed_ln_bwd.argtypes = [vp] * 15 + [i32, i32, i32, i32, i32, i64, i64, i32, i32, f32, u64, u32, vp, sz, vp]
        L.nbest_embed_ln_fwd_interp.argtypes = [vp] * 12 + [i32, i32, i32, f32, i32, f32, u64, u32, vp]
        L.nbest_embed_attrib.argtypes = [vp] * 11 + [i32, i32, i32, i32, f32, i32, vp]
        L.nbest_attention_fwd.argtypes = [vp] * 4 + [i32] * 5 + [f32, u64, u32, vp]
        L.nbest_attention_bwd.argtypes = [vp] * 7 + [i32, vp, sz] + [i32] * 5 + [f32, u64, u32, vp]
        L.nbest_attention_bwd_ws_bytes.argtypes = [i32, i32, i32]
        L.nbest_attention_keep_bytes.argtypes = [i32, i32, i32]
        L.nbest_attention_fwd_keep.argtypes = [vp] * 4 + [i32] * 5 + [f32, u64, u32, vp, vp]
        L.nbest_attention_bwd_keep.argtypes = [vp] * 7 + [i32, vp, sz] + [i32] * 5 + [f32, u64, u32, vp, vp]
        L.nbest_layernorm_fwd.argtypes = [vp] * 5 + [i64, i32, f32, i32, vp]
        L.nbest_layernorm_bwd.argtypes = [vp] * 9 + [i64, i32, i32, i32, f32, u64, u32, vp, sz, vp]
        L.nbest_colsum.argtypes = [vp, vp, i64, i64, i64, i32, i32, vp, sz, vp]
        L.nbest_stc_heads.argtypes = [vp, i64, vp, vp, C.POINTER(LabelSpaceC)] + [vp] * 8 + [i32] * 5 + [f32, u64, u32, vp, sz, vp]
        L.nbest_stc_heads_vjp.argtypes = [vp, C.POINTER(LabelSpaceC)] + [vp] * 8 + [i32, i32, i32, f32, u64, u32, vp, sz, vp]
        L.nbest_cls_mse.argtypes = [vp, i64, vp, i64, vp, vp, vp, i32, i32, i32, f32, vp]
        L.nbest_cls_grad_scatter.argtypes = [vp, vp, i32, i32, i32, i32, vp]
        L.nbest_stc_decode.argtypes = [vp, vp, C.POINTER(LabelSpaceC), vp, vp, i32, vp]
        L.nbest_stream_stamp.argtypes = [vp, i32, vp]
        L.nbest_fp8_amax_fold.argtypes = [vp, vp, i32, vp]
        L.nbest_bertadam_step.argtypes = [vp] * 6 + [i32, i32, f32, f32, f32, f32, f32, vp, sz, vp]
        L.nbest_bertadam_norms.argtypes = [vp, vp, i32, i32, i32, i32, vp, vp]
        L.nbest_bertadam_update.argtypes = [vp] * 6 + [i32, i32, i32, i32, vp, vp, f32, f32, f32, f32, f32, vp]
        L.nbest_adam_clip_coef.argtypes = [vp, i32, f32, vp, vp]
        f64 = C.c_double
        L.nbest_adam_update.argtypes = [i32] + [vp] * 6 + [i32, i32, i32, i32, vp, f32, f32, f32, f64, f64, f32, vp]
        L.nbest_adam_step.argtypes = [i32] + [vp] * 6 + [i32, i32, f32, f32, f32, f64, f64, f32, f32, vp, sz, vp]
        L.nbest_cast_f32_to_bf16.argtypes = [vp, vp, i64, vp]
        L.nbest_encoder_forward.argtypes = [C.POINTER(EncoderDesc)] + [vp] * 7 + [sz, vp, sz, C.POINTER(C.c_void_p), vp]
        L.nbest_encoder_infer_ws_bytes.argtypes = [C.POINTER(EncoderDesc)]
        L.nbest_encoder_infer.argtypes = [C.POINTER(EncoderDesc)] + [vp] * 7 + [sz, vp, vp]
        L.nbest_attention_cls_fwd.argtypes = [vp, i64, vp, i64, vp, vp, i64, i32, i32, i32, i32, i32, vp]
        L.nbest_encoder_infer_attn.argtypes = [C.POINTER(EncoderDesc)] + [vp] * 7 + [sz, vp, vp, vp]
        L.nbest_encoder_act_view.argtypes = [C.POINTER(EncoderDesc), vp, i32, C.POINTER(C.c_void_p), C.POINTER(C.c_void_p)]
        L.nbest_attention_probs.argtypes = [vp] * 4 + [i32] * 5 + [vp]
        L.nbest_attention_cls_probs.argtypes = [vp, i64, vp, i64, vp, vp, i64, i32, i32, i32, i32, i32, vp]
        L.nbest_encoder_backward.argtypes = [C.POINTER(EncoderDesc)] + [vp] * 9 + [sz, vp, vp, sz, i32, i32, i32, i32, vp]
        L.nbest_transpose_weights.argtypes = [vp, vp, vp, i32, i32, vp]
        L.nbest_pack_bn.argtypes = [i64]
        L.nbest_pack_weights.argtypes = [vp, vp, vp, i32, i32, vp]
        L.nbest_pack_bn_fp8.argtypes = [i64, i64]
        L.nbest_pack_weights_fp8.argtypes = [vp, vp, vp, i32, i32, vp]
        L.nbest_gemm_fp8.argtypes = [C.POINTER(GemmFp8Args), vp]
        L.nbest_cast_bf16_to_fp8.argtypes = [vp, vp, i64, vp]
        L.nbest_wgrad_fp8_ws_bytes.restype = C.c_size_t
        L.nbest_wgrad_fp8_ws_bytes.argtypes = [i64, i64, i64]
        L.nbest_wgrad_fp8.argtypes = [vp, vp, vp, i64, i64, i64, i64, i64, i64, vp, vp, i32, vp, sz, vp]
        L.nbest_wgrad_fp8_pair_ws_bytes.restype = C.c_size_t
        L.nbest_wgrad_fp8_pair_ws_bytes.argtypes = [i64, i64, i64, i64]
        L.nbest_wgrad_fp8_pair.argtypes = [vp, vp, vp, i64, i64, i64, i64, vp, vp, vp, vp, vp, i64, i64, i64, i64, vp, vp, i64, i64, i32, vp, sz, vp]
        L.nbest_quantize_weights_fp8.argtypes = [vp, vp, vp, vp, i32, i32, vp, vp, sz, vp]
        L.nbest_gemm_fp8_ws_bytes.restype = C.c_size_t
        L.nbest_gemm_fp8_ws_bytes.argtypes = [C.POINTER(GemmFp8Args)]
        L.nbest_last_error.argtypes = [C.c_char_p, sz]
        _lib = L
    return _lib


def last_error():
    buf = C.create_string_buffer(512)
    lib().nbest_last_error(buf, 512)
    return buf.value.decode(errors="replace")


def check(rc, what):
    if rc != 0:
        raise RuntimeError("nbest_hip %s failed (%d): %s" % (what, rc, last_error()))


def stream_ptr():
    return C.c_void_p(torch.cuda.current_stream().cuda_stream)


def dtype_code(t):
    if t == torch.float32:
        return F32
    if t == torch.bfloat16:
        return BF16
    raise RuntimeError("nbest_amd: unsupported activation dtype %s" % t)


def ptr(t):
    return C.c_void_p(0) if t is None else C.c_void_p(t.data_ptr())


def _ws(nbytes, device):
    return torch.empty(max(int(nbytes), 16), dtype=torch.uint8, device=device)


def gemm_prepared(A, B, M, N, K, out, trans_a=False, trans_b=False, epilogue=EPI_NONE, defer_reduce=False):
    g = GemmArgs()
    g.A, g.B, g.C = A.data_ptr(), B.data_ptr(), out.data_ptr()
    g.M, g.N, g.K = M, N, K
    g.lda, g.ldb, g.ldc = A.stride(0), B.stride(0), out.stride(0)
    g.trans_a, g.trans_b, g.epilogue, g.dtype = int(trans_a), int(trans_b), epilogue, dtype_code(A.dtype)
    g.flags = 1 if defer_reduce else 0
    ws = _ws(lib().nbest_gemm_ws_bytes(C.byref(g)), A.device)
    g.ws, g.ws_bytes = ws.data_ptr(), ws.numel()
    fn, ref, st = lib().nbest_gemm, C.byref(g), stream_ptr()

    def launch():
        rc = fn(ref, st)
        if rc:
            check(rc, "gemm")
    launch.keepalive = (g, ws, A, B, out)
    return launch


def pack_weight(W):
    N, K = W.shape
    bn = lib().nbest_pack_bn(N)
    if bn == 0 or K % 32 or N % bn:
        return None, 0
    d = (MatrixDesc * 1)()
    d[0].offset, d[0].rows, d[0].cols, d[0].tile_start, d[0].pad = 0, N, K, 0, bn
    dd = torch.frombuffer(bytearray(bytes(d)), dtype=torch.uint8).to(W.device)
    out = torch.empty_like(W)
    check(lib().nbest_pack_weights(ptr(W), ptr(out), ptr(dd), 1, (N // bn) * (K // 32), stream_ptr()), "pack_weights")
    return out, bn


def pack_weight_fp8(W8):
    N, K = W8.shape
    bn = lib().nbest_pack_bn_fp8(N, K)
    if bn == 0 or K % 64 or N % bn:
        return None, 0
    d = (MatrixDesc * 1)()
    d[0].offset, d[0].rows, d[0].cols, d[0].tile_start, d[0].pad = 0, N, K, 0, bn
    dd = torch.frombuffer(bytearray(bytes(d)), dtype=torch.uint8).to(W8.device)
    out = torch.empty_like(W8)
    check(lib().nbest_pack_weights_fp8(ptr(W8), ptr(out), ptr(dd), 1, (N // bn) * (K // 64), stream_ptr()), "pack_weights_fp8")
    return out, bn


def gemm(A, B, M, N, K, trans_a=False, trans_b=False, epilogue=EPI_NONE, bias=None, R=None, U=None, out=None,
         accumulate=False, drop_p=0.0, seed=0, drop_stream=0, colsum_out=None, defer_reduce=False, B_packed=None, b_pack_bn=0,
         want_u=True):
    dt = dtype_code(A.dtype)
    dev = A.device
    if out is None:
        out = torch.empty(M, N, dtype=torch.float32 if epilogue == EPI_F32_SPLITK else A.dtype, device=dev)
    if epilogue == EPI_BIAS_GELU and U is None and want_u:
        U = torch.empty(M, N, dtype=torch.float32 if A.dtype == torch.float32 else torch.uint8, device=dev)
    g = GemmArgs()
    g.A, g.B, g.C = A.data_ptr(), B.data_ptr(), out.data_ptr()
    g.bias = bias.data_ptr() if bias is not None else None
    g.R = R.data_ptr() if R is not None else None
    g.U = U.data_ptr() if U is not None else None
    g.M, g.N, g.K = M, N, K
    g.lda, g.ldb, g.ldc = A.stride(0), B.stride(0), out.stride(0)
    g.ldr = R.stride(0) if R is not None else 0
    g.ldu = U.stride(0) if U is not None else 0
    g.trans_a, g.trans_b, g.epilogue, g.dtype = int(trans_a), int(trans_b), epilogue, dt
    g.accumulate, g.drop_p, g.drop_stream, g.seed = int(accumulate), drop_p, drop_stream, seed
    g.colsum_out = colsum_out.data_ptr() if colsum_out is not None else None
    g.flags = 1 if defer_reduce else 0
    if B_packed is not None:
        g.B_packed, g.b_pack_bn = B_packed.data_ptr(), b_pack_bn
    nb = lib().nbest_gemm_ws_bytes(C.byref(g))
    ws = _ws(nb, dev)
    g.ws, g.ws_bytes = ws.data_ptr(), ws.numel()
    check(lib().nbest_gemm(C.byref(g), stream_ptr()), "gemm")
    return (out, U) if epilogue == EPI_BIAS_GELU and want_u else out


def wgrad_pair(dY1, X1, dY2, X2, out1=None, out2=None, accumulate=False):
    K, N = X1.shape
    outs, gs = [], []
    for dY, X, out in ((dY1, X1, out1), (dY2, X2, out2)):
        M = dY.shape[1]
        if out is None:
            out = torch.empty(M, N, dtype=torch.float32, device=X.device)
        g = GemmArgs()
        g.A, g.B, g.C = dY.data_ptr(), X.data_ptr(), out.data_ptr()
        g.M, g.N, g.K = M, N, K
        g.lda, g.ldb, g.ldc = dY.stride(0), X.stride(0), out.stride(0)
        g.trans_a = g.trans_b = 1
        g.epilogue, g.dtype, g.accumulate = EPI_F32_SPLITK, dtype_code(X.dtype), int(accumulate)
        outs.append(out)
        gs.append(g)
    nb = lib().nbest_wgrad_pair_ws_bytes(C.byref(gs[0]), C.byref(gs[1]))
    ws = _ws(nb, X1.device)
    gs[0].ws, gs[0].ws_bytes = ws.data_ptr(), ws.numel()
    check(lib().nbest_wgrad_pair(C.byref(gs[0]), C.byref(gs[1]), stream_ptr()), "wgrad_pair")
    return outs


WGRAD_GROUP_PLAN, WGRAD_GROUP_NEVER, WGRAD_GROUP_ALWAYS = 0, 1, 2


def wgrad_group(problems, outs=None, accumulate=False):
    n = len(problems)
    gs = (GemmArgs * max(n, 1))()
    res = []
    for i, (dY, X) in enumerate(problems):
        M, N = dY.shape[1], X.shape[1]
        out = outs[i] if outs is not None else torch.empty(M, N, dtype=torch.float32, device=X.device)
        g = gs[i]
        g.A, g.B, g.C = dY.data_ptr(), X.data_ptr(), out.data_ptr()
        g.M, g.N, g.K = M, N, X.shape[0]
        g.lda, g.ldb, g.ldc = dY.stride(0), X.stride(0), out.stride(0)
        g.trans_a = g.trans_b = 1
        g.epilogue, g.dtype, g.accumulate = EPI_F32_SPLITK, dtype_code(X.dtype), int(accumulate)
        res.append(out)
    check(lib().nbest_wgrad_group(gs, n, stream_ptr()), "wgrad_group")
    return res


def rows_gather(table, rows, cap):
    H = table.shape[1]
    ids = torch.empty(cap, dtype=torch.long, device=table.device)
    vals = torch.empty(cap, H, dtype=torch.float32, device=table.device)
    check(lib().nbest_rows_gather(ptr(table), ptr(rows), rows.numel(), cap, ptr(ids), ptr(vals), H, stream_ptr()), "rows_gather")
    return ids, vals


def rows_zero(table, ids):
    check(lib().nbest_rows_zero(ptr(table), ptr(ids), ids.numel(), table.shape[1], stream_ptr()), "rows_zero")


def rows_add(table, ids, vals):
    check(lib().nbest_rows_add(ptr(table), ptr(ids), ptr(vals), ids.numel(), table.shape[1], stream_ptr()), "rows_add")


def gelu_d_decode(U):
    return U if U.dtype == torch.float32 else (U.float() - 26.0) / 200.0


def gelu_d_encode(g):
    return torch.clamp(torch.round(g.float() * 200.0 + 26.0), 0, 255).to(torch.uint8)


def cast_fp8(x):
    out = torch.empty(x.shape, dtype=torch.uint8, device=x.device)
    check(lib().nbest_cast_bf16_to_fp8(ptr(x), ptr(out), x.numel(), stream_ptr()), "cast_bf16_to_fp8")
    return out


def gemm_fp8(A8, W8, M, N, K, bias, out_scale=1.0, epilogue=EPI_BIAS, R=None, drop_p=0.0, seed=0, drop_stream=0, out=None, B_packed=None, b_pack_bn=0):
    dev = A8.device
    if out is None:
        out = torch.empty(M, N, dtype=torch.bfloat16, device=dev)
    g = GemmFp8Args()
    g.A, g.B, g.C, g.bias = A8.data_ptr(), W8.data_ptr(), out.data_ptr(), bias.data_ptr()
    g.M, g.N, g.K, g.lda, g.ldb, g.ldc = M, N, K, A8.stride(0), W8.stride(0), out.stride(0)
    g.epilogue, g.out_scale, g.drop_p, g.drop_stream, g.seed = epilogue, out_scale, drop_p, drop_stream, seed
    U = C8 = None
    if epilogue == EPI_BIAS_GELU:
        U = torch.empty(M, N, dtype=torch.uint8, device=dev)
        C8 = torch.empty(M, N, dtype=torch.uint8, device=dev)
        g.U, g.C8, g.ldu, g.ldc8 = U.data_ptr(), C8.data_ptr(), N, N
    if R is not None:
        g.R, g.ldr = R.data_ptr(), R.stride(0)
    if B_packed is not None:
        g.B_packed, g.b_pack_bn = B_packed.data_ptr(), b_pack_bn
    check(lib().nbest_gemm_fp8(C.byref(g), stream_ptr()), "gemm_fp8")
    return (out, U, C8) if epilogue == EPI_BIAS_GELU else out


def wgrad_fp8(dY8, X8, M, N, K, a_amax=None, out=None, accumulate=False, x_amax=None):
    if out is None:
        out = torch.zeros(M, N, dtype=torch.float32, device=dY8.device)
    ws = _ws(lib().nbest_wgrad_fp8_ws_bytes(M, N, K), dY8.device)
    check(lib().nbest_wgrad_fp8(ptr(dY8), ptr(X8), ptr(out), M, N, K, dY8.stride(0), X8.stride(0), out.stride(0), ptr(a_amax), ptr(x_amax),
                                int(accumulate), ptr(ws), ws.numel(), stream_ptr()), "wgrad_fp8")
    return out


def wgrad_fp8_pair(dY8a, X8a, dY8b, X8b, amax_a=None, amax_b=None, outs=None, accumulate=False, xamax_a=None, xamax_b=None):
    K, N = X8a.shape
    Ma, Mb = dY8a.shape[1], dY8b.shape[1]
    oa, ob = outs if outs is not None else (torch.zeros(Ma, N, dtype=torch.float32, device=X8a.device),
                                            torch.zeros(Mb, N, dtype=torch.float32, device=X8a.device))
    ws = _ws(lib().nbest_wgrad_fp8_pair_ws_bytes(Ma, Mb, N, K), X8a.device)
    check(lib().nbest_wgrad_fp8_pair(ptr(dY8a), ptr(X8a), ptr(oa), Ma, dY8a.stride(0), X8a.stride(0), oa.stride(0), ptr(amax_a), ptr(xamax_a),
                                     ptr(dY8b), ptr(X8b), ptr(ob), Mb, dY8b.stride(0), X8b.stride(0), ob.stride(0), ptr(amax_b), ptr(xamax_b),
                                     N, K, int(accumulate), ptr(ws), ws.numel(), stream_ptr()), "wgrad_fp8_pair")
    return oa, ob


def layernorm_fwd(x, gamma, beta, eps):
    M, H = x.shape
    y = torch.empty_like(x)
    stats = torch.empty(M, 2, dtype=torch.float32, device=x.device)
    check(lib().nbest_layernorm_fwd(ptr(x), ptr(gamma), ptr(beta), ptr(y), ptr(stats), M, H, eps, dtype_code(x.dtype),
                                    stream_ptr()), "layernorm_fwd")
    return y, stats


def layernorm_bwd(dy, x, stats, gamma, want_dbias=True, drop_p=0.0, seed=0, drop_stream=0):
    M, H = x.shape
    dx = torch.empty_like(x)
    dxd = torch.empty_like(x) if drop_p > 0 else None
    dg = torch.zeros(H, dtype=torch.float32, device=x.device)
    db = torch.zeros_like(dg)
    dbias = torch.zeros_like(dg) if want_dbias else None
    ws = _ws(lib().nbest_rowred_ws_bytes(M, H), x.device)
    check(lib().nbest_layernorm_bwd(ptr(dy), ptr(x), ptr(stats), ptr(gamma), ptr(dx), ptr(dxd), ptr(dg), ptr(db), ptr(dbias),
                                    M, H, dtype_code(x.dtype), 0, drop_p, seed, drop_stream, ptr(ws), ws.numel(), stream_ptr()),
          "layernorm_bwd")
    return dx, dxd, dg, db, dbias


def colsum(X, accumulate=False, out=None):
    M, N = X.shape
    if out is None:
        out = torch.zeros(N, dtype=torch.float32, device=X.device)
    ws = _ws(lib().nbest_rowred_ws_bytes(M, N), X.device)
    check(lib().nbest_colsum(ptr(X), ptr(out), M, N, X.stride(0), dtype_code(X.dtype), int(accumulate), ptr(ws), ws.numel(),
                             stream_ptr()), "colsum")
    return out


def attention_fwd(qkv, key_mask, B, S, heads, drop_p=0.0, seed=0, drop_stream=0, want_keep=False):
    H = heads * 64
    ctx = torch.empty(B * S, H, dtype=qkv.dtype, device=qkv.device)
    lse = torch.empty(B, heads, S, dtype=torch.float32, device=qkv.device)
    if want_keep:
        nb = lib().nbest_attention_keep_bytes(B, S, heads) if qkv.dtype == torch.bfloat16 else 0
        keep = torch.zeros(nb // 4, dtype=torch.int32, device=qkv.device) if nb else None
        check(lib().nbest_attention_fwd_keep(ptr(qkv), ptr(key_mask), ptr(ctx), ptr(lse), B, S, heads, 64, dtype_code(qkv.dtype),
                                             drop_p, seed, drop_stream, ptr(keep), stream_ptr()), "attention_fwd_keep")
        return ctx, lse, keep
    check(lib().nbest_attention_fwd(ptr(qkv), ptr(key_mask), ptr(ctx), ptr(lse), B, S, heads, 64, dtype_code(qkv.dtype),
                                    drop_p, seed, drop_stream, stream_ptr()), "attention_fwd")
    return ctx, lse


def attention_cls_fwd(q, ldq, kv, ldkv, key_mask, B, S, heads, out=None):
    H = heads * 64
# ... 209 lines not shown
```

n-best-asr-transformer_amd/optim.py:

```python
import torch
import torch.distributed as dist

from . import hipabi as hb
from .model import freeze_plan


def warmup_linear(step, t_total, warmup):
    if t_total < 0:
        return 1.0
    x = float(step) / float(t_total)
    if x < warmup:
        return x / warmup
    return max((x - 1.0) / (warmup - 1.0), 0.0)


class HipBertAdam:

    def __init__(self, model, lr, bert_lr=None, warmup=-1, t_total=-1, b1=0.9, b2=0.999, e=1e-6, max_grad_norm=1.0, shard=False):
        self.model, self.arena = model, model.arena
        self.lr, self.bert_lr = lr, lr if bert_lr is None else bert_lr
        self.warmup, self.t_total = max(warmup, 0.0), t_total
        self.b1, self.b2, self.e, self.max_grad_norm = b1, b2, e, max_grad_norm
        self.step_count = 0
        a = self.arena
        self._frozen_key = None
        self._trainable = None
        if hasattr(model, "_params"):
            plan = freeze_plan(model)
            self._frozen_key, self._trainable = plan.key, plan.trainable
        if a.m is None:
            a.m = torch.zeros_like(a.p)
            a.v = torch.zeros_like(a.p)
        is_emb = lambda name: name.startswith("bert_encoder.embeddings.")
        self.parts = []
        self._selects = (lambda n: not is_emb(n), is_emb)
        for sel in self._selects:
            descs, n_t, n_b = self._build_descs(sel)
            ws = torch.empty((n_b + n_t + 16) * 4, dtype=torch.uint8, device=a.device)
            self.parts.append((descs, n_t, n_b, ws))
        self.rank, self.world = 0, 1
        if dist.is_available() and dist.is_initialized():
            self.rank, self.world = dist.get_rank(), dist.get_world_size()
        self.sharded = bool(shard) and self.world > 1 and getattr(a, "w8", None) is None
        self.owner_ranges = None
        if self.sharded:
            self._plan_shards()

    def _plan_shards(self):
        a, W = self.arena, self.world
        self.blk_bounds, self.elem_ranges, self.small_idx, self.partials, self.coefs = [], [], [], [], []
        for part, sel in enumerate(self._selects):
            blocks = a.block_table(sel, self._active())
            n_t, n_b = self.parts[part][1], self.parts[part][2]
            assert len(blocks) == n_b, (len(blocks), n_b)
            weight = [n if act else 0 for _, n, act in blocks]
            total, acc, cuts = sum(weight), 0, [0]
            for i, w in enumerate(weight):
                acc += w
                while len(cuts) < W and acc * W >= total * len(cuts):
                    cuts.append(i + 1)
            while len(cuts) < W:
                cuts.append(n_b)
            cuts.append(n_b)
            bb = [(cuts[r], max(cuts[r], cuts[r + 1])) for r in range(W)]
            er = [(blocks[lo][0], blocks[hi - 1][0] + blocks[hi - 1][1]) if hi > lo else (0, 0) for lo, hi in bb]
            self.blk_bounds.append(bb)
            self.elem_ranges.append(er)
            idx = []
            smalls = a.fp32_read_slots(sel)
            for r, (lo, hi) in enumerate(er):
                pieces = [torch.arange(max(s.offset, lo), min(s.offset + s.numel, hi), dtype=torch.long) for s in smalls
                          if min(s.offset + s.numel, hi) > max(s.offset, lo)]
                idx.append((torch.cat(pieces) if pieces else torch.empty(0, dtype=torch.long)).to(a.device))
            self.small_idx.append(idx)
            self.partials.append(torch.zeros(max(n_b, 1), dtype=torch.float32, device=a.device))
            self.coefs.append(torch.zeros(max(n_t, 1), dtype=torch.float32, device=a.device))
        self.owner_ranges = [[self.elem_ranges[p_][r] for p_ in range(len(self.parts)) if self.elem_ranges[p_][r][1] > self.elem_ranges[p_][r][0]]
                             for r in range(W)]

    def _build_descs(self, select):
        return self.arena.build_descs(self.lr, self.bert_lr, select=select, active=self._active())

    def _active(self):
        t = self._trainable
        return None if t is None else (lambda n: n in t)

    def sync_frozen(self):
        if not hasattr(self.model, "_params"):
            return False
        plan = freeze_plan(self.model)
        if plan.key == self._frozen_key:
            return False
        self._frozen_key, self._trainable = plan.key, plan.trainable
        for part, sel in enumerate(self._selects):
            descs, n_t, n_b = self._build_descs(sel)
            assert (n_t, n_b) == self.parts[part][1:3]
            self.parts[part] = (descs, n_t, n_b, self.parts[part][3])
        if self.sharded:
            self.gather_master()
            old = self.owner_ranges
            self._plan_shards()
            old[:] = self.owner_ranges
            self.owner_ranges = old
        return True

    def get_lr_mult(self):
        return warmup_linear(self.step_count, self.t_total, self.warmup)

    def zero_grad(self):
        self.arena.g.zero_()

    def _launch(self, part):
        a = self.arena
        descs, n_t, n_b, ws = self.parts[part]
        if n_t == 0:
            return
        if self.sharded:
            return self._launch_sharded(part)
        hb.check(hb.lib().nbest_bertadam_step(hb.ptr(a.p), hb.ptr(a.g), hb.ptr(a.m), hb.ptr(a.v), hb.ptr(a.w16),
                                              hb.ptr(descs), n_t, n_b, self.get_lr_mult(),
                                              self.b1, self.b2, self.e, self.max_grad_norm, hb.ptr(ws),
                                              ws.numel(), hb.stream_ptr()), "bertadam_step")

    def _launch_sharded(self, part):
        a = self.arena
        descs, n_t, n_b, _ = self.parts[part]
        lo, hi = self.blk_bounds[part][self.rank]
        partial, coef = self.partials[part], self.coefs[part]
        partial.zero_()
        hb.check(hb.lib().nbest_bertadam_norms(hb.ptr(a.g), hb.ptr(descs), n_t, n_b, lo, hi, hb.ptr(partial), hb.stream_ptr()), "bertadam_norms")
        dist.all_reduce(partial, op=dist.ReduceOp.SUM)
        hb.check(hb.lib().nbest_bertadam_update(hb.ptr(a.p), hb.ptr(a.g), hb.ptr(a.m), hb.ptr(a.v), hb.ptr(a.w16), hb.ptr(descs), n_t, n_b,
                                                lo, hi, hb.ptr(partial), hb.ptr(coef), self.get_lr_mult(), self.b1, self.b2, self.e,
                                                self.max_grad_norm, hb.stream_ptr()), "bertadam_update")
        self._broadcast_owned(part)

    def _broadcast_owned(self, part):
        a = self.arena
        for r, (elo, ehi) in enumerate(self.elem_ranges[part]):
            if ehi <= elo:
                continue
            if a.w16 is None:
                dist.broadcast(a.p[elo:ehi], src=r)
                continue
            dist.broadcast(a.w16[elo:ehi], src=r)
            idx = self.small_idx[part][r]
            if idx.numel():
                buf = a.p.index_select(0, idx) if r == self.rank else torch.empty(idx.numel(), dtype=torch.float32, device=a.device)
                dist.broadcast(buf, src=r)
                if r != self.rank:
                    a.p.index_copy_(0, idx, buf)

    def gather_master(self, moments=True):
        if not self.sharded:
            return
        a = self.arena
        for part in range(len(self.parts)):
            for r, (elo, ehi) in enumerate(self.elem_ranges[part]):
                if ehi > elo:
                    dist.broadcast(a.p[elo:ehi], src=r)
                    if moments:
                        dist.broadcast(a.m[elo:ehi], src=r)
                        dist.broadcast(a.v[elo:ehi], src=r)

    def step_main(self):
        self.sync_frozen()
        self._launch(0)
        self.arena.refresh_transposed()

    def step_embeddings(self):
        self._launch(1)
        self.step_count += 1

    def step(self):
        self.step_main()
        self.step_embeddings()

    def state_dict(self, gather=True):
        if gather:
            self.gather_master()
        a = self.arena
        return dict(step=self.step_count, t_total=self.t_total, warmup=self.warmup,
                    state={s.name: dict(next_m=a.view(a.m, s.name).detach().cpu().clone(),
                                        next_v=a.view(a.v, s.name).detach().cpu().clone()) for s in a.slots})

    def load_state_dict(self, sd):
        if sd.get("kind", "bertadam") != "bertadam":
            raise ValueError("optimizer state of kind %r cannot be loaded into BertAdam (--optim_choice must match the run that "
                             "wrote it)" % sd["kind"])
        a = self.arena
        self.step_count = int(sd["step"])
        for s in a.slots:
            st = sd["state"][s.name]
            a.view(a.m, s.name).copy_(st["next_m"])
            a.view(a.v, s.name).copy_(st["next_v"])


def linear_schedule_with_warmup(k, warmup_steps, t_total):
    if k < warmup_steps:
        return float(k) / float(max(1, warmup_steps))
    return max(0.0, float(t_total - k) / float(max(1, t_total - warmup_steps)))


class LinearScheduleWithWarmup:

    def __init__(self, warmup_steps, t_total):
        self.warmup_steps, self.t_total, self.last_epoch = int(warmup_steps), int(t_total), 0

    def get_lr_mult(self):
        return linear_schedule_with_warmup(self.last_epoch, self.warmup_steps, self.t_total)

    def step(self):
        self.last_epoch += 1


class HipAdam(HipBertAdam):

    KINDS = {"adam": hb.ADAM_L2, "adamw": hb.ADAMW}

    def __init__(self, model, kind="adamw", lr=5e-4, bert_lr=None, l2=0.0, warmup=0.0, t_total=-1, max_grad_norm=5.0, shard=False,
                 b1=0.9, b2=0.999):
        if kind not in self.KINDS:
            raise ValueError("HipAdam: kind must be 'adam' or 'adamw', not %r" % (kind,))
        self.kind, self.mode, self.l2 = kind, self.KINDS[kind], float(l2)
        if kind == "adam":
            bert_lr = lr
        super().__init__(model, lr, bert_lr=bert_lr, warmup=warmup, t_total=t_total, b1=b1, b2=b2,
                         e=1e-8 if kind == "adam" else 1e-6, max_grad_norm=max_grad_norm, shard=shard)
        self.scheduler = None
        if kind == "adamw":
            self.scheduler = LinearScheduleWithWarmup(int(self.warmup * t_total), t_total)
        self.blk_base = [0, self.parts[0][2]]
        self.partial = torch.zeros(max(self.parts[0][2] + self.parts[1][2], 1), dtype=torch.float32, device=self.arena.device)
        self.clip = torch.ones(2, dtype=torch.float32, device=self.arena.device)

    def _build_descs(self, select):
        if self.kind == "adam":
            return self.arena.build_descs(self.lr, self.lr, select=select, wd=self.l2, active=self._active())
        return self.arena.build_descs(self.lr, self.bert_lr, select=select, active=self._active())

    def get_lr_mult(self):
        return 1.0 if self.scheduler is None else self.scheduler.get_lr_mult()

    def _range(self, part):
        return self.blk_bounds[part][self.rank] if self.sharded else (0, self.parts[part][2])

    def _norms(self, part):
        a = self.arena
        descs, n_t, n_b, _ = self.parts[part]
        if n_t == 0 or self.max_grad_norm <= 0:
            return
        lo, hi = self._range(part)
        hb.check(hb.lib().nbest_bertadam_norms(hb.ptr(a.g), hb.ptr(descs), n_t, n_b, lo, hi, hb.ptr(self.partial[self.blk_base[part]:]),
                                               hb.stream_ptr()), "bertadam_norms")

    def step_main(self):
        self.sync_frozen()
        if self.sharded and self.max_grad_norm > 0:
            self.partial.zero_()
        self._norms(0)

    def step_embeddings(self):
        a = self.arena
        self._norms(1)
        if self.max_grad_norm > 0:
            if self.sharded:
                dist.all_reduce(self.partial, op=dist.ReduceOp.SUM)
            hb.check(hb.lib().nbest_adam_clip_coef(hb.ptr(self.partial), self.partial.numel(), self.max_grad_norm, hb.ptr(self.clip),
                                                   hb.stream_ptr()), "adam_clip_coef")
        else:
            self.clip.fill_(1.0)
        t = self.step_count + 1
        bc1, bc2s = (1.0 - self.b1 ** t, (1.0 - self.b2 ** t) ** 0.5) if self.kind == "adam" else (1.0, 1.0)
        lr_mult = self.get_lr_mult()
        for part in range(len(self.parts)):
            descs, n_t, n_b, _ = self.parts[part]
            if n_t == 0:
                continue
            lo, hi = self._range(part)
            hb.check(hb.lib().nbest_adam_update(self.mode, hb.ptr(a.p), hb.ptr(a.g), hb.ptr(a.m), hb.ptr(a.v), hb.ptr(a.w16), hb.ptr(descs),
                                                n_t, n_b, lo, hi, hb.ptr(self.clip), lr_mult, bc1, bc2s, self.b1, self.b2, self.e,
                                                hb.stream_ptr()), "adam_update")
        if self.sharded:
            for part in range(len(self.parts)):
                self._broadcast_owned(part)
        a.refresh_transposed()
        self.step_count += 1

    def state_dict(self, gather=True):
        if gather:
            self.gather_master()
        a = self.arena
        return dict(kind=self.kind, step=self.step_count, sched_step=None if self.scheduler is None else self.scheduler.last_epoch,
                    t_total=self.t_total, warmup=self.warmup,
                    state={s.name: dict(exp_avg=a.view(a.m, s.name).detach().cpu().clone(),
                                        exp_avg_sq=a.view(a.v, s.name).detach().cpu().clone()) for s in a.slots})

    def load_state_dict(self, sd):
        kind = sd.get("kind", "bertadam")
        if kind != self.kind:
            raise ValueError("optimizer state of kind %r cannot be loaded into HipAdam(kind=%r) (--optim_choice must match the run "
                             "that wrote it)" % (kind, self.kind))
        a = self.arena
        self.step_count = int(sd["step"])
        if self.scheduler is not None:
            self.scheduler.last_epoch = int(sd["sched_step"])
        for s in a.slots:
            st = sd["state"][s.name]
            a.view(a.m, s.name).copy_(st["exp_avg"])
            a.view(a.v, s.name).copy_(st["exp_avg_sq"])
```

Baseline: 12780.

## Fuse optimizer update with bf16, transposed and packed weight image generation

```diff
diff --git a/include/nbest_hip.h b/include/nbest_hip.h
--- a/include/nbest_hip.h
+++ b/include/nbest_hip.h
@@ -226,6 +226,24 @@
 int nbest_pack_bn_fp8(int64_t N, int64_t K);
 int nbest_pack_weights_fp8(const void* src, void* dst, const nbest_matrix_desc* descs, int n_matrices, int n_stages, nbest_stream_t stream);
 int nbest_pack_weights(const void* src, void* dst, const nbest_matrix_desc* descs, int n_matrices, int n_stages, nbest_stream_t stream);
+typedef struct nbest_optim_matrix_desc {
+  int64_t offset;
+  int32_t rows, cols;
+  int32_t row0, nrows;
+  int32_t tile_start;
+  int32_t tensor;
+} nbest_optim_matrix_desc;
+int nbest_weight_tile(void);
+int nbest_weight_images(const void* w16, void* w16t, void* wpk, void* wpkt, const nbest_optim_matrix_desc* mdescs, int n_matrices,
+                        int n_tiles, nbest_stream_t stream);
+int nbest_bertadam_step_images(float* p, float* g, float* m, float* v, void* w16, void* w16t, void* wpk, void* wpkt,
+                               const nbest_tensor_desc* descs, int n_tensors, int n_blocks, const nbest_optim_matrix_desc* mdescs,
+                               int n_matrices, int n_tiles, float lr_mult, float b1, float b2, float eps, float max_grad_norm,
+                               void* ws, size_t ws_bytes, nbest_stream_t stream);
+int nbest_adam_update_images(int mode, float* p, const float* g, float* m, float* v, void* w16, void* w16t, void* wpk, void* wpkt,
+                             const nbest_tensor_desc* descs, int n_tensors, int n_blocks, const nbest_optim_matrix_desc* mdescs,
+                             int n_matrices, int n_tiles, const float* clip, float lr_mult, float bc1, float bc2_sqrt, double b1,
+                             double b2, float eps, nbest_stream_t stream);
 int nbest_cast_f32_to_bf16(const float* src, void* dst, int64_t n, nbest_stream_t stream);
 
 typedef struct nbest_layer_offsets {
diff --git a/n-best-asr-transformer_amd/arena.py b/n-best-asr-transformer_amd/arena.py
--- a/n-best-asr-transformer_amd/arena.py
+++ b/n-best-asr-transformer_amd/arena.py
@@ -44,6 +44,7 @@
             add(pre + n, enc[n])
         self.layer_offsets = (hb.LayerOffsets * cfg.num_hidden_layers)()
         self.layer_range = []
+        self.matrix_tensors = []
         for i in range(cfg.num_hidden_layers):
             lp = "encoder.layer.%d." % i
             lo = None
@@ -63,6 +64,12 @@
                               ("ln2_g", "output.LayerNorm.weight"), ("ln2_b", "output.LayerNorm.bias")):
                 setattr(o, field, add(pre + lp + nm, enc[lp + nm]).offset)
             self.layer_range.append((lo, off))
+            H_, F_ = cfg.hidden_size, cfg.intermediate_size
+            for j, nm in enumerate(("query", "key", "value")):
+                self.matrix_tensors.append((o.wqkv, 3 * H_, H_, j * H_, H_, pre + lp + "attention.self.%s.weight" % nm))
+            for moff, r, c, nm in ((o.wo, H_, H_, "attention.output.dense.weight"), (o.w1, F_, H_, "intermediate.dense.weight"),
+                                   (o.w2, H_, F_, "output.dense.weight")):
+                self.matrix_tensors.append((moff, r, c, 0, r, pre + lp + nm))
         add(pre + "pooler.dense.weight", enc["pooler.dense.weight"])
         add(pre + "pooler.dense.bias", enc["pooler.dense.bias"])
         heads = head_param_shapes(labels, cfg.hidden_size)
@@ -95,6 +102,7 @@
         self.wpk = self.wpkt = None
         self.w8p = self.w8tp = None
         self._pdescs = None
+        self._idescs = None
         if self.w16 is not None and self.device.type == "cuda":
             self.w16t = torch.zeros(self.total, dtype=torch.bfloat16, device=self.device)
             H, F = cfg.hidden_size, cfg.intermediate_size
@@ -129,7 +137,23 @@
             if self._pdescs is not None:
                 self.wpk = torch.zeros(self.total, dtype=torch.bfloat16, device=self.device)
                 self.wpkt = torch.zeros(self.total, dtype=torch.bfloat16, device=self.device)
+            self._idescs = self.image_descs()
         self._descs = None
+
+    def image_descs(self, tensor_index=None):
+        tile = hb.lib().nbest_weight_tile()
+        arr = (hb.OptimMatrixDesc * max(len(self.matrix_tensors), 1))()
+        t = 0
+        for i, (off, r, c, row0, nrows, name) in enumerate(self.matrix_tensors):
+            if r % tile or c % tile or row0 % tile or nrows % tile or off % 8:
+                return None
+            d = arr[i]
+            d.offset, d.rows, d.cols, d.row0, d.nrows, d.tile_start = off, r, c, row0, nrows, t
+            d.tensor = -1 if tensor_index is None else tensor_index(name)
+            t += (nrows // tile) * (c // tile)
+        if not self.matrix_tensors:
+            return None
+        return torch.frombuffer(bytearray(bytes(arr)), dtype=torch.uint8).to(self.device), len(self.matrix_tensors), t
 
     def view(self, buf, name):
         s = self.by_name[name]
@@ -152,8 +176,8 @@
             hb.cast_bf16(self.p, self.w16)
         self.refresh_transposed()
 
-    def refresh_transposed(self):
-        if self.w16t is not None:
+    def refresh_transposed(self, bf16=True):
+        if self.w16t is not None and bf16:
             if self.lazy_w16t:
                 self.w16t_stale = True
             else:
@@ -168,6 +192,12 @@
                     hb.check(hb.lib().nbest_pack_weights_fp8(hb.ptr(src), hb.ptr(dst), hb.ptr(pd), pn, pt, hb.stream_ptr()), "pack_weights_fp8")
 
     def refresh_w16t(self):
+        if self._idescs is not None:
+            d, n, t = self._idescs
+            hb.check(hb.lib().nbest_weight_images(hb.ptr(self.w16), hb.ptr(self.w16t), hb.ptr(self.wpk), hb.ptr(self.wpkt), hb.ptr(d), n, t,
+                                                  hb.stream_ptr()), "weight_images")
+            self.w16t_stale = False
+            return
         d, n, t = self._tdescs
         hb.check(hb.lib().nbest_transpose_weights(hb.ptr(self.w16), hb.ptr(self.w16t), hb.ptr(d), n, t, hb.stream_ptr()),
                  "transpose_weights")
diff --git a/n-best-asr-transformer_amd/csrc/common.h b/n-best-asr-transformer_amd/csrc/common.h
--- a/n-best-asr-transformer_amd/csrc/common.h
+++ b/n-best-asr-transformer_amd/csrc/common.h
@@ -157,6 +157,19 @@
   }
 }
 
+__host__ __device__ __forceinline__ int nb_pack_bn(int64_t N) {
+  if (N % 256 == 0 && N >= 1024) return 256;
+  if (N % 192 == 0) return 192;
+  return 0;
+}
+__device__ __forceinline__ int64_t nb_pack_chunk(int R, int c, int K, int bn) {
+  const int pw = (bn == 256) ? 128 : 96, q = pw / 16, nk = K >> 5;
+  const int tile_n = R / bn, g = R - tile_n * bn, blk = g / pw, y = g - blk * pw;
+  const int row = blk * pw + (y / q) + 16 * (y % q);
+  const int slot = (c & 3) ^ ((-(row >> 2)) & 3);
+  return (((int64_t)tile_n * nk + (c >> 2)) * bn + row) * 4 + slot;
+}
+
 __device__ __forceinline__ float wave_sum(float v) {
 #pragma unroll
   for (int o = 32; o > 0; o >>= 1) v += __shfl_xor(v, o, 64);
diff --git a/n-best-asr-transformer_amd/csrc/gemm_bf16_v2.hip b/n-best-asr-transformer_amd/csrc/gemm_bf16_v2.hip
--- a/n-best-asr-transformer_amd/csrc/gemm_bf16_v2.hip
+++ b/n-best-asr-transformer_amd/csrc/gemm_bf16_v2.hip
@@ -1111,11 +1111,7 @@
   return NBEST_OK;
 }
 
-int nbest_pack_bn_internal(int64_t N) {
-  if (N % 256 == 0 && N >= 1024) return 256;
-  if (N % 192 == 0) return 192;
-  return 0;
-}
+int nbest_pack_bn_internal(int64_t N) { return nb_pack_bn(N); }
 
 int nbest_pack_weights_bf16(const void* src, void* dst, const nbest_matrix_desc* descs, int n_matrices, int n_stages, hipStream_t st) {
   pack_b_kernel<<<n_stages, 256, 0, st>>>((const bf16*)src, (bf16*)dst, descs, n_matrices);
diff --git a/n-best-asr-transformer_amd/csrc/optim.hip b/n-best-asr-transformer_amd/csrc/optim.hip
--- a/n-best-asr-transformer_amd/csrc/optim.hip
+++ b/n-best-asr-transformer_amd/csrc/optim.hip
@@ -55,6 +55,15 @@
   }
 }
 
+__device__ __forceinline__ bool is_tiled_tensor(const nbest_optim_matrix_desc* __restrict__ md, int n, int t) {
+  int lo = 0, hi = n - 1;
+  while (lo < hi) {
+    const int mid = (lo + hi + 1) >> 1;
+    if (md[mid].tensor <= t) lo = mid; else hi = mid - 1;
+  }
+  return n > 0 && md[lo].tensor == t;
+}
+
 __device__ __forceinline__ void adam1(float& p, float g, float& m, float& v, float coef, float b1, float b2, float eps,
                                       float lr, float wd) {
   g *= coef;
@@ -69,11 +78,11 @@
                                                        float* __restrict__ v, bf16* __restrict__ plow,
                                                        const nbest_tensor_desc* __restrict__ descs, int n_tensors,
                                                        const float* __restrict__ coef, float lr_mult, float b1, float b2, float eps,
-                                                       int blk_off) {
+                                                       int blk_off, const nbest_optim_matrix_desc* __restrict__ tiled, int n_tiled) {
   const int blk = blockIdx.x + blk_off;
   const int t = find_tensor(descs, n_tensors, blk);
   const nbest_tensor_desc d = descs[t];
-  if (!d.active) return;
+  if (!d.active || is_tiled_tensor(tiled, n_tiled, t)) return;
   const float cf = coef[t];
   const float lr = d.lr * lr_mult;
   const int64_t c0 = (int64_t)(blk - d.block_start) * kChunk;
@@ -149,11 +158,12 @@
                                                    float* __restrict__ v, bf16* __restrict__ plow,
                                                    const nbest_tensor_desc* __restrict__ descs, int n_tensors,
                                                    const float* __restrict__ clip, float lr_mult, float bc1, float bc2s, float b1,
-                                                   float b2, float ob1, float ob2, float eps, int blk_off) {
+                                                   float b2, float ob1, float ob2, float eps, int blk_off,
+                                                   const nbest_optim_matrix_desc* __restrict__ tiled, int n_tiled) {
   const int blk = blockIdx.x + blk_off;
   const int t = find_tensor(descs, n_tensors, blk);
   const nbest_tensor_desc d = descs[t];
-  if (!d.active) return;
+  if (!d.active || is_tiled_tensor(tiled, n_tiled, t)) return;
   const float cf = clip[0];
   const float lr = d.lr * lr_mult / bc1;
   const int64_t c0 = (int64_t)(blk - d.block_start) * kChunk;
@@ -217,6 +227,118 @@
   }
 }
 
+constexpr int kWT = 64;
+constexpr int kWP = kWT + 8;
+constexpr int kWC = kWT / 8;
+constexpr int kWI = kWT * kWC / 256;
+static_assert(kWC == 8, "the chunk swizzle of the transposed LDS image is written for 8 chunks per row");
+
+__device__ __forceinline__ int find_matrix(const nbest_optim_matrix_desc* __restrict__ md, int n, int tile) {
+  int lo = 0, hi = n - 1;
+  while (lo < hi) {
+    const int mid = (lo + hi + 1) >> 1;
+    if (md[mid].tile_start <= tile) lo = mid; else hi = mid - 1;
+  }
+  return lo;
+}
+
+__device__ __forceinline__ void write_weight_images(const bf16* tile, bf16* tt, const nbest_optim_matrix_desc& md, int r0, int c0,
+                                                    bf16* __restrict__ w16, bf16* __restrict__ w16t, bf16* __restrict__ wpk,
+                                                    bf16* __restrict__ wpkt) {
+  const int bn = nb_pack_bn(md.rows), bnt = nb_pack_bn(md.cols);
+  if (bn == 0) wpk = nullptr;
+  if (bnt == 0) wpkt = nullptr;
+  const bool tr = w16t || wpkt;
+#pragma unroll
+  for (int it = 0; it < kWI; ++it) {
+    const int idx = it * 256 + threadIdx.x, r = idx / kWC, ch = idx % kWC;
+    const bf16x8 x = *(const bf16x8*)(tile + r * kWP + ch * 8);
+    const int R = r0 + r, Cc = c0 + ch * 8;
+    if (w16) *(bf16x8*)(w16 + md.offset + (int64_t)R * md.cols + Cc) = x;
+    if (wpk) *(bf16x8*)(wpk + md.offset + nb_pack_chunk(R, Cc >> 3, md.cols, bn) * 8) = x;
+    if (tr) {
+#pragma unroll
+      for (int e = 0; e < 8; ++e) tt[(ch * 8 + e) * kWP + (((r >> 3) ^ ch) << 3) + (r & 7)] = x[e];
+    }
+  }
+  if (!tr) return;
+  __syncthreads();
+#pragma unroll
+  for (int it = 0; it < kWI; ++it) {
+    const int idx = it * 256 + threadIdx.x, c = idx / kWC, ch = idx % kWC;
+    const bf16x8 x = *(const bf16x8*)(tt + c * kWP + ((ch ^ ((c >> 3) % kWC)) << 3));
+    const int R = c0 + c, Cc = r0 + ch * 8;
+    if (w16t) *(bf16x8*)(w16t + md.offset + (int64_t)R * md.rows + Cc) = x;
+    if (wpkt) *(bf16x8*)(wpkt + md.offset + nb_pack_chunk(R, Cc >> 3, md.rows, bnt) * 8) = x;
+  }
+}
+
+__global__ __launch_bounds__(256) void weight_images_kernel(const bf16* __restrict__ w16, bf16* __restrict__ w16t, bf16* __restrict__ wpk,
+                                                            bf16* __restrict__ wpkt, const nbest_optim_matrix_desc* __restrict__ mdescs,
+                                                            int n_mats) {
+  __shared__ __attribute__((aligned(16))) bf16 tile[kWT * kWP];
+  __shared__ __attribute__((aligned(16))) bf16 tt[kWT * kWP];
+  const nbest_optim_matrix_desc md = mdescs[find_matrix(mdescs, n_mats, blockIdx.x)];
+  const int t = blockIdx.x - md.tile_start, tc = md.cols / kWT;
+  const int r0 = md.row0 + (t / tc) * kWT, c0 = (t % tc) * kWT;
+#pragma unroll
+  for (int it = 0; it < kWI; ++it) {
+    const int idx = it * 256 + threadIdx.x, r = idx / kWC, ch = idx % kWC;
+    *(bf16x8*)(tile + r * kWP + ch * 8) = *(const bf16x8*)(w16 + md.offset + (int64_t)(r0 + r) * md.cols + c0 + ch * 8);
+  }
+  __syncthreads();
+  write_weight_images(tile, tt, md, r0, c0, nullptr, w16t, wpk, wpkt);
+}
+
+constexpr int kBertAdam = 2;
+struct TileUpdP {
+  float lr_mult, bc1, bc2s, b1, b2, ob1, ob2, eps;
+};
+
+template <int MODE>
+__global__ __launch_bounds__(256) void optim_tile_kernel(float* __restrict__ p, const float* __restrict__ g, float* __restrict__ m,
+                                                         float* __restrict__ v, bf16* __restrict__ w16, bf16* __restrict__ w16t,
+                                                         bf16* __restrict__ wpk, bf16* __restrict__ wpkt,
+                                                         const nbest_tensor_desc* __restrict__ descs,
+                                                         const nbest_optim_matrix_desc* __restrict__ mdescs, int n_mats,
+                                                         const float* __restrict__ coef, TileUpdP a) {
+  __shared__ __attribute__((aligned(16))) bf16 tile[kWT * kWP];
+  __shared__ __attribute__((aligned(16))) bf16 tt[kWT * kWP];
+  const nbest_optim_matrix_desc md = mdescs[find_matrix(mdescs, n_mats, blockIdx.x)];
+  const nbest_tensor_desc d = descs[md.tensor];
+  if (!d.active) return;
+  const float cf = coef[MODE == kBertAdam ? md.tensor : 0];
+  const float lr = (MODE == kBertAdam) ? d.lr * a.lr_mult : d.lr * a.lr_mult / a.bc1;
+  const int t = blockIdx.x - md.tile_start, tc = md.cols / kWT;
+  const int r0 = md.row0 + (t / tc) * kWT, c0 = (t % tc) * kWT;
+#pragma unroll
+  for (int it = 0; it < kWI; ++it) {
+    const int idx = it * 256 + threadIdx.x, r = idx / kWC, ch = idx % kWC;
+    const int64_t o = md.offset + (int64_t)(r0 + r) * md.cols + c0 + ch * 8;
+    bf16x8 lowp;
+#pragma unroll
+    for (int h = 0; h < 2; ++h) {
+      const int64_t i = o + 4 * h;
+      f32x4 pp = *(f32x4*)(p + i), gg = *(const f32x4*)(g + i);
+      f32x4 mm = *(f32x4*)(m + i), vv = *(f32x4*)(v + i);
+#pragma unroll
+      for (int e = 0; e < 4; ++e) {
+        float p1 = pp[e], m1 = mm[e], v1e = vv[e];
+        if (MODE == kBertAdam) adam1(p1, gg[e], m1, v1e, cf, a.b1, a.b2, a.eps, lr, d.wd);
+        else adam_mode1<MODE == kBertAdam ? NBEST_ADAMW : MODE>(p1, gg[e], m1, v1e, cf, a.b1, a.b2, a.ob1, a.ob2, a.eps, lr, d.wd, a.bc2s);
+        pp[e] = p1; mm[e] = m1; vv[e] = v1e;
+        lowp[4 * h + e] = (bf16)p1;
+      }
+      *(f32x4*)(p + i) = pp;
+      *(f32x4*)(m + i) = mm;
+      *(f32x4*)(v + i) = vv;
+    }
+    *(bf16x8*)(tile + r * kWP + ch * 8) = lowp;
+  }
+  __syncthreads();
+  write_weight_images(tile, tt, md, r0, c0, w16, w16t, wpk, wpkt);
+}
+
 }
 
 extern "C" int nbest_transpose_weights(const void* src, void* dst, const nbest_matrix_desc* descs, int n_matrices, int n_tiles,
@@ -248,7 +370,7 @@
   clip_coef_kernel<<<n_tensors, 64, 0, st>>>(partial, descs, n_tensors, n_blocks, max_grad_norm, coef);
   NB_LAUNCH_CHECK();
   if (blk_hi == blk_lo) return NBEST_OK;
-  bertadam_kernel<<<blk_hi - blk_lo, 256, 0, st>>>(p, g, m, v, (bf16*)p_lowp, descs, n_tensors, coef, lr_mult, b1, b2, eps, blk_lo);
+  bertadam_kernel<<<blk_hi - blk_lo, 256, 0, st>>>(p, g, m, v, (bf16*)p_lowp, descs, n_tensors, coef, lr_mult, b1, b2, eps, blk_lo, nullptr, 0);
   NB_LAUNCH_CHECK();
   return NBEST_OK;
 }
@@ -282,10 +404,10 @@
   const float fb1 = (float)b1, fb2 = (float)b2, ob1 = (float)(1.0 - b1), ob2 = (float)(1.0 - b2);
   if (mode == NBEST_ADAM_L2)
     adam_kernel<NBEST_ADAM_L2><<<blk_hi - blk_lo, 256, 0, st>>>(p, g, m, v, (bf16*)p_lowp, descs, n_tensors, clip, lr_mult, bc1,
-                                                                bc2_sqrt, fb1, fb2, ob1, ob2, eps, blk_lo);
+                                                                bc2_sqrt, fb1, fb2, ob1, ob2, eps, blk_lo, nullptr, 0);
   else
     adam_kernel<NBEST_ADAMW><<<blk_hi - blk_lo, 256, 0, st>>>(p, g, m, v, (bf16*)p_lowp, descs, n_tensors, clip, lr_mult, bc1,
-                                                              bc2_sqrt, fb1, fb2, ob1, ob2, eps, blk_lo);
+                                                              bc2_sqrt, fb1, fb2, ob1, ob2, eps, blk_lo, nullptr, 0);
   NB_LAUNCH_CHECK();
   return NBEST_OK;
 }
@@ -302,3 +424,62 @@
   return nbest_adam_update(mode, p, g, m, v, p_lowp, descs, n_tensors, n_blocks, 0, n_blocks, clip, lr_mult, bc1, bc2_sqrt, b1, b2, eps,
                            stream);
 }
+
+extern "C" int nbest_weight_tile(void) { return kWT; }
+
+extern "C" int nbest_weight_images(const void* w16, void* w16t, void* wpk, void* wpkt, const nbest_optim_matrix_desc* mdescs,
+                                   int n_matrices, int n_tiles, nbest_stream_t stream) {
+  NB_CHECK(w16 && mdescs && n_matrices > 0 && n_tiles > 0 && (w16t || wpk || wpkt), NBEST_ERR_ARG, "weight_images: bad arguments");
+  weight_images_kernel<<<n_tiles, 256, 0, (hipStream_t)stream>>>((const bf16*)w16, (bf16*)w16t, (bf16*)wpk, (bf16*)wpkt, mdescs,
+                                                                 n_matrices);
+  NB_LAUNCH_CHECK();
+  return NBEST_OK;
+}
+
+extern "C" int nbest_bertadam_step_images(float* p, float* g, float* m, float* v, void* w16, void* w16t, void* wpk, void* wpkt,
+                                          const nbest_tensor_desc* descs, int n_tensors, int n_blocks,
+                                          const nbest_optim_matrix_desc* mdescs, int n_matrices, int n_tiles, float lr_mult, float b1,
+                                          float b2, float eps, float max_grad_norm, void* ws, size_t ws_bytes, nbest_stream_t stream) {
+  NB_CHECK(p && g && m && v && w16 && descs && mdescs && ws && n_tensors > 0 && n_blocks > 0 && n_matrices > 0 && n_tiles > 0,
+           NBEST_ERR_ARG, "bertadam_step_images: bad arguments");
+  NB_CHECK(ws_bytes >= ((size_t)n_blocks + n_tensors) * sizeof(float), NBEST_ERR_WORKSPACE, "bertadam_step_images: workspace too small");
+  hipStream_t st = (hipStream_t)stream;
+  float* partial = (float*)ws;
+  float* coef = partial + n_blocks;
+  if (int rc = nbest_bertadam_norms(g, descs, n_tensors, n_blocks, 0, n_blocks, partial, stream)) return rc;
+  clip_coef_kernel<<<n_tensors, 64, 0, st>>>(partial, descs, n_tensors, n_blocks, max_grad_norm, coef);
+  NB_LAUNCH_CHECK();
+  bertadam_kernel<<<n_blocks, 256, 0, st>>>(p, g, m, v, (bf16*)w16, descs, n_tensors, coef, lr_mult, b1, b2, eps, 0, mdescs, n_matrices);
+  NB_LAUNCH_CHECK();
+  const TileUpdP a = {lr_mult, 1.f, 1.f, b1, b2, 0.f, 0.f, eps};
+  optim_tile_kernel<kBertAdam><<<n_tiles, 256, 0, st>>>(p, g, m, v, (bf16*)w16, (bf16*)w16t, (bf16*)wpk, (bf16*)wpkt, descs, mdescs,
+                                                        n_matrices, coef, a);
+  NB_LAUNCH_CHECK();
+  return NBEST_OK;
+}
+
+extern "C" int nbest_adam_update_images(int mode, float* p, const float* g, float* m, float* v, void* w16, void* w16t, void* wpk,
+                                        void* wpkt, const nbest_tensor_desc* descs, int n_tensors, int n_blocks,
+                                        const nbest_optim_matrix_desc* mdescs, int n_matrices, int n_tiles, const float* clip,
+                                        float lr_mult, float bc1, float bc2_sqrt, double b1, double b2, float eps, nbest_stream_t stream) {
+  NB_CHECK(p && g && m && v && w16 && descs && mdescs && clip && n_tensors > 0 && n_blocks > 0 && n_matrices > 0 && n_tiles > 0 &&
+           (mode == NBEST_ADAM_L2 || mode == NBEST_ADAMW) && bc1 > 0.f && bc2_sqrt > 0.f, NBEST_ERR_ARG, "adam_update_images: bad arguments");
+  hipStream_t st = (hipStream_t)stream;
+  const float fb1 = (float)b1, fb2 = (float)b2, ob1 = (float)(1.0 - b1), ob2 = (float)(1.0 - b2);
+  const TileUpdP a = {lr_mult, bc1, bc2_sqrt, fb1, fb2, ob1, ob2, eps};
+  if (mode == NBEST_ADAM_L2) {
+    adam_kernel<NBEST_ADAM_L2><<<n_blocks, 256, 0, st>>>(p, g, m, v, (bf16*)w16, descs, n_tensors, clip, lr_mult, bc1, bc2_sqrt, fb1, fb2,
+                                                         ob1, ob2, eps, 0, mdescs, n_matrices);
+    NB_LAUNCH_CHECK();
+    optim_tile_kernel<NBEST_ADAM_L2><<<n_tiles, 256, 0, st>>>(p, g, m, v, (bf16*)w16, (bf16*)w16t, (bf16*)wpk, (bf16*)wpkt, descs, mdescs,
+                                                              n_matrices, clip, a);
+  } else {
+    adam_kernel<NBEST_ADAMW><<<n_blocks, 256, 0, st>>>(p, g, m, v, (bf16*)w16, descs, n_tensors, clip, lr_mult, bc1, bc2_sqrt, fb1, fb2,
+                                                       ob1, ob2, eps, 0, mdescs, n_matrices);
+    NB_LAUNCH_CHECK();
+    optim_tile_kernel<NBEST_ADAMW><<<n_tiles, 256, 0, st>>>(p, g, m, v, (bf16*)w16, (bf16*)w16t, (bf16*)wpk, (bf16*)wpkt, descs, mdescs,
+                                                            n_matrices, clip, a);
+  }
+  NB_LAUNCH_CHECK();
+  return NBEST_OK;
+}
diff --git a/n-best-asr-transformer_amd/hipabi.py b/n-best-asr-transformer_amd/hipabi.py
--- a/n-best-asr-transformer_amd/hipabi.py
+++ b/n-best-asr-transformer_amd/hipabi.py
@@ -21,6 +21,7 @@
     "nbest_attention_cls_fwd", "nbest_encoder_infer_ws_bytes", "nbest_encoder_infer",
     "nbest_attention_probs", "nbest_attention_cls_probs", "nbest_encoder_act_view", "nbest_encoder_infer_attn",
     "nbest_embed_ln_fwd_interp", "nbest_embed_attrib",
+    "nbest_weight_tile", "nbest_weight_images", "nbest_bertadam_step_images", "nbest_adam_update_images",
 ]
 
 
@@ -57,6 +58,11 @@
 
 class MatrixDesc(C.Structure):
     _fields_ = [("offset", C.c_int64), ("rows", C.c_int32), ("cols", C.c_int32), ("tile_start", C.c_int32), ("pad", C.c_int32)]
+
+
+class OptimMatrixDesc(C.Structure):
+    _fields_ = [("offset", C.c_int64), ("rows", C.c_int32), ("cols", C.c_int32), ("row0", C.c_int32), ("nrows", C.c_int32),
+                ("tile_start", C.c_int32), ("tensor", C.c_int32)]
 
 
 class LayerOffsets(C.Structure):
@@ -140,6 +146,9 @@
         f64 = C.c_double
         L.nbest_adam_update.argtypes = [i32] + [vp] * 6 + [i32, i32, i32, i32, vp, f32, f32, f32, f64, f64, f32, vp]
         L.nbest_adam_step.argtypes = [i32] + [vp] * 6 + [i32, i32, f32, f32, f32, f64, f64, f32, f32, vp, sz, vp]
+        L.nbest_weight_images.argtypes = [vp, vp, vp, vp, vp, i32, i32, vp]
+        L.nbest_bertadam_step_images.argtypes = [vp] * 9 + [i32, i32, vp, i32, i32, f32, f32, f32, f32, f32, vp, sz, vp]
+        L.nbest_adam_update_images.argtypes = [i32] + [vp] * 9 + [i32, i32, vp, i32, i32, vp, f32, f32, f32, f64, f64, f32, vp]
         L.nbest_cast_f32_to_bf16.argtypes = [vp, vp, i64, vp]
         L.nbest_encoder_forward.argtypes = [C.POINTER(EncoderDesc)] + [vp] * 7 + [sz, vp, sz, C.POINTER(C.c_void_p), vp]
         L.nbest_encoder_infer_ws_bytes.argtypes = [C.POINTER(EncoderDesc)]
diff --git a/n-best-asr-transformer_amd/optim.py b/n-best-asr-transformer_amd/optim.py
--- a/n-best-asr-transformer_amd/optim.py
+++ b/n-best-asr-transformer_amd/optim.py
@@ -16,7 +16,8 @@
 
 class HipBertAdam:
 
-    def __init__(self, model, lr, bert_lr=None, warmup=-1, t_total=-1, b1=0.9, b2=0.999, e=1e-6, max_grad_norm=1.0, shard=False):
+    def __init__(self, model, lr, bert_lr=None, warmup=-1, t_total=-1, b1=0.9, b2=0.999, e=1e-6, max_grad_norm=1.0, shard=False,
+                 fuse_images=True):
         self.model, self.arena = model, model.arena
         self.lr, self.bert_lr = lr, lr if bert_lr is None else bert_lr
         self.warmup, self.t_total = max(warmup, 0.0), t_total
@@ -38,6 +39,9 @@
             descs, n_t, n_b = self._build_descs(sel)
             ws = torch.empty((n_b + n_t + 16) * 4, dtype=torch.uint8, device=a.device)
             self.parts.append((descs, n_t, n_b, ws))
+        self.fuse_images = bool(fuse_images)
+        index = {s.name: i for i, s in enumerate(s_ for s_ in a.slots if self._selects[0](s_.name))}
+        self._images = a.image_descs(index.__getitem__) if a.w16t is not None else None
         self.rank, self.world = 0, 1
         if dist.is_available() and dist.is_initialized():
             self.rank, self.world = dist.get_rank(), dist.get_world_size()
@@ -110,13 +114,25 @@
     def zero_grad(self):
         self.arena.g.zero_()
 
-    def _launch(self, part):
+    def _fused(self):
+        a = self.arena
+        return (self.fuse_images and not self.sharded and self._images is not None and a.w16 is not None and a.w16t is not None
+                and not a.lazy_w16t and not a.w16t_stale)
+
+    def _launch(self, part, fused=False):
         a = self.arena
         descs, n_t, n_b, ws = self.parts[part]
         if n_t == 0:
             return
         if self.sharded:
             return self._launch_sharded(part)
+        if fused and part == 0:
+            md, n_m, n_tiles = self._images
+            hb.check(hb.lib().nbest_bertadam_step_images(hb.ptr(a.p), hb.ptr(a.g), hb.ptr(a.m), hb.ptr(a.v), hb.ptr(a.w16), hb.ptr(a.w16t),
+                                                         hb.ptr(a.wpk), hb.ptr(a.wpkt), hb.ptr(descs), n_t, n_b, hb.ptr(md), n_m, n_tiles,
+                                                         self.get_lr_mult(), self.b1, self.b2, self.e, self.max_grad_norm, hb.ptr(ws),
+                                                         ws.numel(), hb.stream_ptr()), "bertadam_step_images")
+            return
         hb.check(hb.lib().nbest_bertadam_step(hb.ptr(a.p), hb.ptr(a.g), hb.ptr(a.m), hb.ptr(a.v), hb.ptr(a.w16),
                                               hb.ptr(descs), n_t, n_b, self.get_lr_mult(),
                                               self.b1, self.b2, self.e, self.max_grad_norm, hb.ptr(ws),
@@ -165,8 +181,9 @@
 
     def step_main(self):
         self.sync_frozen()
-        self._launch(0)
-        self.arena.refresh_transposed()
+        fused = self._fused()
+        self._launch(0, fused)
+        self.arena.refresh_transposed(bf16=not fused)
 
     def step_embeddings(self):
         self._launch(1)
@@ -219,14 +236,14 @@
     KINDS = {"adam": hb.ADAM_L2, "adamw": hb.ADAMW}
 
     def __init__(self, model, kind="adamw", lr=5e-4, bert_lr=None, l2=0.0, warmup=0.0, t_total=-1, max_grad_norm=5.0, shard=False,
-                 b1=0.9, b2=0.999):
+                 b1=0.9, b2=0.999, fuse_images=True):
         if kind not in self.KINDS:
             raise ValueError("HipAdam: kind must be 'adam' or 'adamw', not %r" % (kind,))
         self.kind, self.mode, self.l2 = kind, self.KINDS[kind], float(l2)
         if kind == "adam":
             bert_lr = lr
         super().__init__(model, lr, bert_lr=bert_lr, warmup=warmup, t_total=t_total, b1=b1, b2=b2,
-                         e=1e-8 if kind == "adam" else 1e-6, max_grad_norm=max_grad_norm, shard=shard)
+                         e=1e-8 if kind == "adam" else 1e-6, max_grad_norm=max_grad_norm, shard=shard, fuse_images=fuse_images)
         self.scheduler = None
         if kind == "adamw":
             self.scheduler = LinearScheduleWithWarmup(int(self.warmup * t_total), t_total)
@@ -273,9 +290,17 @@
         t = self.step_count + 1
         bc1, bc2s = (1.0 - self.b1 ** t, (1.0 - self.b2 ** t) ** 0.5) if self.kind == "adam" else (1.0, 1.0)
         lr_mult = self.get_lr_mult()
+        fused = self._fused()
         for part in range(len(self.parts)):
             descs, n_t, n_b, _ = self.parts[part]
             if n_t == 0:
+                continue
+            if fused and part == 0:
+                md, n_m, n_tiles = self._images
+                hb.check(hb.lib().nbest_adam_update_images(self.mode, hb.ptr(a.p), hb.ptr(a.g), hb.ptr(a.m), hb.ptr(a.v), hb.ptr(a.w16),
+                                                           hb.ptr(a.w16t), hb.ptr(a.wpk), hb.ptr(a.wpkt), hb.ptr(descs), n_t, n_b, hb.ptr(md),
+                                                           n_m, n_tiles, hb.ptr(self.clip), lr_mult, bc1, bc2s, self.b1, self.b2, self.e,
+                                                           hb.stream_ptr()), "adam_update_images")
                 continue
             lo, hi = self._range(part)
             hb.check(hb.lib().nbest_adam_update(self.mode, hb.ptr(a.p), hb.ptr(a.g), hb.ptr(a.m), hb.ptr(a.v), hb.ptr(a.w16), hb.ptr(descs),
@@ -284,7 +309,7 @@
         if self.sharded:
             for part in range(len(self.parts)):
                 self._broadcast_owned(part)
-        a.refresh_transposed()
+        a.refresh_transposed(bf16=not fused)
         self.step_count += 1
 
     def state_dict(self, gather=True):
```

Measured after the change: 12770 (median of 2 runs). Within noise of the previous version (-0.1%).
